# cebarker1000/heatflow

Measured on AMD Instinct MI355X. Metric: DOF-updates/s (timesteps/s x nDOF) on geballe_with_diamond, higher is better.
Workload: dtype f64

## Files before the change

heatflow_amd/csrc/heatflow_hip.hip:

```cpp

#include "hf_amg_io.hpp"

namespace {

struct MeshTables {
  std::vector<int32_t> rowptr, colidx;
  ColDict spmv;
  RowGather rg;
  std::vector<char> tag_used;
  int max_blk_nnz = 0;
};

constexpr char BLOB_MAGIC[8] = {'H', 'F', 'P', 'A', 'T', '0', '2', 0};
struct BlobHeader {
  char magic[8];
  int64_t total_bytes, nnz;
  int32_t n, ne, rba, ts, max_blk_nnz, tab_len, rg_ok, rg_max_dict, spmv_max_dict, reserved;
  int64_t count[12];
};

void steady_swap(hf_ctx* ctx) {
  hf_ctx::Steady& S = ctx->steady;
  std::swap(ctx->nbc, S.nbc); std::swap(ctx->d_bc_dofs, S.bc_dofs); std::swap(ctx->d_g, S.g);
  std::swap(ctx->nlift_rows, S.nlift_rows); std::swap(ctx->nlift, S.nlift);
// ... 393 lines not shown
  HF_TRY(dev_alloc(ctx, &F.part_rz, 2 * static_cast<size_t>(nv) * MAXP));
  HF_TRY(dev_alloc(ctx, &F.part_zz, static_cast<size_t>(nv) * MAXP));
  HF_TRY(dev_alloc(ctx, &F.part_bn, static_cast<size_t>(nv) * MAXP));
  HF_TRY(dev_alloc(ctx, &F.scal, nv));
  HF_TRY(dev_alloc(ctx, &F.red, 1));
  HF_HIP(hipMemsetAsync(F.scal, 0, sizeof(Scal) * nv, ctx->stream));
  HF_HIP(hipMemsetAsync(F.red, 0, sizeof(BRed), ctx->stream));
  if (hipHostMalloc(reinterpret_cast<void**>(&F.h_scal), sizeof(Scal) * nv) != hipSuccess) return fail(ctx, HF_ERR_ALLOC, "hipHostMalloc failed");
  const int rpb = TPB / nv;
  F.Pb = static_cast<int>(std::min<size_t>((static_cast<size_t>(ctx->n) + rpb - 1) / rpb, MAXP));
  if (F.Pb >= 64) F.Pb &= ~7;
  F.opk = 0; F.pred_iters = 0;
  F.sysA = ctx->d_M1; F.sysDinv = ctx->d_dinv1;
  F.lds = ctx->bcols.nv == nv;
  HF_HIP(hipStreamSynchronize(ctx->stream));
  F.nv = nv;
  return HF_OK;
}

int batch_flux_step(hf_ctx* ctx, int components, double rtol, int max_it, int nfs, double* out, int32_t* it_out) {
  hf_ctx::Batch& B = ctx->batch;
  hf_ctx::Batch& F = ctx->fluxnb;
  const int nv = B.nv;
  const int capd = ctx->rg_max_dict;
  const size_t sm = static_cast<size_t>(capd) * 16 + static_cast<size_t>(capd + (capd & 1)) * 8 + (RBA + 4) * 4 +
                    (static_cast<size_t>((ctx->max_blk_nnz + 1) & ~1) / 8 + 3) * 16;
  const int grid = std::min(ctx->nblk_a, 2048);
  int done = 0;
  for (int comp = 0; comp < 2; ++comp) {
    if (!((components >> comp) & 1)) continue;
    const bool second = done == 1;
    if (second) std::swap(F.u, F.uprev);
    for (int j = 0; j < nv; ++j)
      hipLaunchKernelGGL(k_grad_rows, dim3(grid), dim3(RBA), sm, ctx->stream, ctx->nblk_a, capd, ctx->d_rg_hdr,
                         reinterpret_cast<const uint4*>(ctx->d_rg_ell), reinterpret_cast<const uint4*>(ctx->d_rg_cid), ctx->d_rg_zrb,
                         ctx->d_rg_dict, ctx->d_rowptr, B.u, comp == 0 ? F.b + j : static_cast<double*>(nullptr),
                         comp == 1 ? F.b + j : static_cast<double*>(nullptr), nv, nv, j);
    HF_HIP(hipGetLastError());
    std::swap(ctx->batch, ctx->fluxnb);
    const int rc = batch_dispatch(ctx, [&](auto ops) { return decltype(ops)::pcg(ctx, false, rtol, 0.0, max_it); });
    int itmax = 0;
    for (int j = 0; j < nv; ++j) itmax = std::max(itmax, ctx->batch.h_scal[j].iters);
    std::swap(ctx->batch, ctx->fluxnb);
    if (it_out) it_out[done] = itmax;
    if (rc != HF_OK) { if (second) std::swap(F.u, F.uprev); return rc; }
    double* o = out + static_cast<size_t>(done) * nv * nfs;
    const int thr = nfs * nv;
    switch (nv) {
      case 2: hipLaunchKernelGGL((kb_gather<2>), dim3((thr + 255) / 256), dim3(256), 0, ctx->stream, nfs, ctx->d_fsamp_idx, F.u, o); break;
      case 4: hipLaunchKernelGGL((kb_gather<4>), dim3((thr + 255) / 256), dim3(256), 0, ctx->stream, nfs, ctx->d_fsamp_idx, F.u, o); break;
      case 8: hipLaunchKernelGGL((kb_gather<8>), dim3((thr + 255) / 256), dim3(256), 0, ctx->stream, nfs, ctx->d_fsamp_idx, F.u, o); break;
      default: hipLaunchKernelGGL((kb_gather<16>), dim3((thr + 255) / 256), dim3(256), 0, ctx->stream, nfs, ctx->d_fsamp_idx, F.u, o); break;
    }
    HF_HIP(hipGetLastError());
    if (second) std::swap(F.u, F.uprev);
    ++done;
  }
  return HF_OK;
}
int tangent_reset(hf_ctx* ctx) {
  hf_ctx::Batch& T = ctx->tanb;
  if (T.nv == 0) return HF_OK;
  HF_HIP(hipMemsetAsync(T.u, 0, sizeof(double) * static_cast<size_t>(ctx->n) * T.nv, ctx->stream));
  HF_HIP(hipStreamSynchronize(ctx->stream));
  T.bdf_hist = false;
  for (bool& u_ : T.pused) u_ = false;
  T.pnext = 0; T.ppending = -1;
  T.pred_iters = 0;
  return HF_OK;
}

int tangent_levels(hf_ctx* ctx) {
  hf_ctx::Batch& T = ctx->tanb;
  std::vector<int64_t> sig;
  if (ctx->precond == 1 && ctx->amg_ready)
    for (const DevLevel& L : ctx->amg) { sig.push_back(L.n); sig.push_back(L.P.ncol); }
  if (sig == ctx->tan.lev_sig) return HF_OK;
  for (auto& L : T.lev) { dev_free(&L.x); dev_free(&L.cat); if (L.own_b) dev_free(&L.b); }
  T.lev.clear();
  HF_TRY(batch_levels(ctx, T, T.nv));
  HF_HIP(hipStreamSynchronize(ctx->stream));
  ctx->tan.lev_sig = sig;
  return HF_OK;
}

int tangent_load(hf_ctx* ctx) {
  const int capd = ctx->rg_max_dict;
  const size_t sm = static_cast<size_t>(capd) * 16 + static_cast<size_t>(capd + (capd & 1)) * 8 + (RBA + 4) * 4 +
                    (static_cast<size_t>((ctx->max_blk_nnz + 1) & ~1) / 8 + 3) * 16;
  const int grid = std::min(ctx->nblk_a, 2048);
#define HF_TL(NV) hipLaunchKernelGGL(k_tangent_load<NV>, dim3(grid), dim3(RBA), sm, ctx->stream, ctx->nblk_a, capd, ctx->d_rg_hdr, \
                                     reinterpret_cast<const uint4*>(ctx->d_rg_ell), reinterpret_cast<const uint4*>(ctx->d_rg_cid), \
                                     ctx->d_rg_zrb, ctx->d_rg_dict, ctx->d_rowptr, ctx->tan.col, ctx->d_u, ctx->tan.F)
  switch (ctx->tan.nv) {
    case 2: HF_TL(2); break;
    case 4: HF_TL(4); break;
    case 8: HF_TL(8); break;
    default: HF_TL(16); break;
  }
#undef HF_TL
  HF_HIP(hipGetLastError());
  return HF_OK;
}

}

extern "C" {

const char* hf_version(void) { return "heatflow_hip 0.1 (gfx950)"; }

const char* hf_last_error(const hf_ctx* ctx) { return ctx ? ctx->err.c_str() : "null context"; }

int hf_create(int device_id, hf_ctx** out) {
  if (!out) return HF_ERR_ARG;
  *out = nullptr;
  int count = 0;
  if (hipGetDeviceCount(&count) != hipSuccess || count <= 0) return HF_ERR_HIP;
  if (device_id < 0 || device_id >= count) return HF_ERR_ARG;
  hf_ctx* ctx = new hf_ctx();
  ctx->dev = device_id;
  auto bail = [&](int rc) { *out = ctx; return rc; };
  if (hipSetDevice(device_id) != hipSuccess) return bail(fail(ctx, HF_ERR_HIP, "hipSetDevice(%d) failed", device_id));
  if (hipStreamCreateWithFlags(&ctx->stream, hipStreamNonBlocking) != hipSuccess)
    return bail(fail(ctx, HF_ERR_HIP, "hipStreamCreate failed"));
  if (hipEventCreate(&ctx->ev0) != hipSuccess || hipEventCreate(&ctx->ev1) != hipSuccess)
    return bail(fail(ctx, HF_ERR_HIP, "hipEventCreate failed"));
  if (hipHostMalloc(reinterpret_cast<void**>(&ctx->h_scal), sizeof(Scal)) != hipSuccess)
    return bail(fail(ctx, HF_ERR_ALLOC, "hipHostMalloc failed"));
  if (hipHostMalloc(reinterpret_cast<void**>(&ctx->h_mirror), sizeof(ScalMirror), hipHostMallocMapped | hipHostMallocCoherent) != hipSuccess ||
      hipHostGetDevicePointer(reinterpret_cast<void**>(&ctx->d_mirror), ctx->h_mirror, 0) != hipSuccess)
    return bail(fail(ctx, HF_ERR_ALLOC, "hipHostMalloc (mapped) failed"));
  *ctx->h_mirror = ScalMirror{};
  int rc = dev_alloc(ctx, &ctx->d_scal, 1);
  if (rc == HF_OK) rc = dev_alloc(ctx, &ctx->d_part_pAp, MAXP);
  if (rc == HF_OK) rc = dev_alloc(ctx, &ctx->d_part_rz, 2 * MAXP);
  if (rc == HF_OK) rc = dev_alloc(ctx, &ctx->d_part_zz, MAXP);
  if (rc == HF_OK) rc = dev_alloc(ctx, &ctx->d_part_bn, MAXP);
  if (rc == HF_OK && reset_scal(ctx) != HF_OK) rc = HF_ERR_HIP;
  if (rc == HF_OK) {
    hipLaunchKernelGGL(k_zero_entries, dim3(1), dim3(64), 0, ctx->stream, 0, static_cast<const int32_t*>(nullptr), static_cast<double*>(nullptr));
    if (hipStreamSynchronize(ctx->stream) != hipSuccess) rc = fail(ctx, HF_ERR_HIP, "first kernel launch failed: %s", hipGetErrorString(hipGetLastError()));
  }
  *out = ctx;
  return rc;
}

int hf_destroy(hf_ctx* ctx) {
  if (!ctx) return HF_ERR_ARG;
  (void)hipSetDevice(ctx->dev);
  if (ctx->stream) (void)hipStreamSynchronize(ctx->stream);
  dev_free(&ctx->d_zr); dev_free(&ctx->d_elem); dev_free(&ctx->d_kappa); dev_free(&ctx->d_rhoc);
  dev_free(&ctx->d_rowptr); dev_free(&ctx->d_colidx); dev_free(&ctx->d_cdict_ptr); dev_free(&ctx->d_cdict); dev_free(&ctx->d_cid); dev_free(&ctx->d_blk_eptr); dev_free(&ctx->d_blk_cptr); dev_free(&ctx->d_blk_ent); dev_free(&ctx->d_rg_hdr); dev_free(&ctx->d_rg_ell); dev_free(&ctx->d_rg_cid); dev_free(&ctx->d_rg_dict); dev_free(&ctx->d_rg_zrb); dev_free(&ctx->d_kappa_rg); dev_free(&ctx->d_rhoc_rg); dev_free(&ctx->d_M); dev_free(&ctx->d_A); dev_free(&ctx->d_dinv);
  dev_free(&ctx->d_bc_dofs); dev_free(&ctx->d_g); dev_free(&ctx->d_lift_rows); dev_free(&ctx->d_lift_ptr);
  dev_free(&ctx->d_lift_bc); dev_free(&ctx->d_lift_slot); dev_free(&ctx->d_lift_val);
  dev_free(&ctx->d_uprev); dev_free(&ctx->d_ustart);
  dev_free(&ctx->d_u); dev_free(&ctx->d_b); dev_free(&ctx->d_r); dev_free(&ctx->d_p); dev_free(&ctx->d_Ap);
  free_batch(ctx); free_batch_state(ctx->fluxb); free_batch_cols(ctx); free_amg(ctx); free_responses(ctx); proj_free(ctx); dev_free(&ctx->d_z); dev_free(&ctx->d_z2);
  steady_free(ctx); load_free(ctx); tangent_free(ctx); kt_free(ctx);
  dev_free(&ctx->d_M1); dev_free(&ctx->d_dinv1); dev_free(&ctx->d_gz); dev_free(&ctx->d_gr); dev_free(&ctx->d_bz); dev_free(&ctx->d_br);
  dev_free(&ctx->d_tmp); dev_free(&ctx->d_part_pAp); dev_free(&ctx->d_part_rz); dev_free(&ctx->d_part_zz);
  dev_free(&ctx->d_part_bn); dev_free(&ctx->d_scal); dev_free(&ctx->d_samp_idx); dev_free(&ctx->d_samp); dev_free(&ctx->d_fsamp_idx);
  for (auto& e : ctx->prof_ev) (void)hipEventDestroy(e);
  if (ctx->h_scal) (void)hipHostFree(ctx->h_scal);
  if (ctx->h_mirror) (void)hipHostFree(ctx->h_mirror);
  if (ctx->ev0) (void)hipEventDestroy(ctx->ev0);
  if (ctx->ev1) (void)hipEventDestroy(ctx->ev1);
  if (ctx->stream) (void)hipStreamDestroy(ctx->stream);
  delete ctx;
  return HF_OK;
}

int hf_set_mesh(hf_ctx* ctx, int32_t n, int32_t ne, const double* zr, const int32_t* tri, const int32_t* tag) {
  if (!ctx) return HF_ERR_ARG;
  if (!zr || !tri || !tag || n <= 0 || ne <= 0) return fail(ctx, HF_ERR_ARG, "hf_set_mesh: null pointer or empty mesh");
  HF_HIP(hipSetDevice(ctx->dev));
  int32_t maxtag = 0;
  for (int64_t k = 0; k < 3LL * ne; ++k)
    if (tri[k] < 0 || tri[k] >= n) return fail(ctx, HF_ERR_ARG, "hf_set_mesh: triangle %lld references node %d outside [0,%d)", (long long)(k / 3), tri[k], n);
  for (int32_t e = 0; e < ne; ++e) {
    if (tag[e] < 0) return fail(ctx, HF_ERR_ARG, "hf_set_mesh: negative cell tag at cell %d", e);
    maxtag = std::max(maxtag, tag[e]);
    const double* p0 = zr + 2 * tri[3 * e], *p1 = zr + 2 * tri[3 * e + 1], *p2 = zr + 2 * tri[3 * e + 2];
    const double d = (p1[0] - p0[0]) * (p2[1] - p0[1]) - (p2[0] - p0[0]) * (p1[1] - p0[1]);
    if (!(d != 0.0)) return fail(ctx, HF_ERR_ARG, "hf_set_mesh: degenerate triangle %d", e);
  }
  const auto t0 = std::chrono::steady_clock::now();
  auto lap = [&](const char* what) {
    if (std::getenv("HEATFLOW_DEBUG")) std::fprintf(stderr, "[set_mesh] %-28s %.3f s\n", what, std::chrono::duration<double>(std::chrono::steady_clock::now() - t0).count());
  };
  lap("checked");
  MeshTables T;
  Pattern P;
  HF_TRY(build_csr(ctx, n, ne, tri, P));
  lap("+ csr pattern");
  build_rowgather(n, ne, tri, tag, P);
  lap("+ row-gather lists");
  if (!build_coldict(P.rowptr, P.colidx, n, SRPC, T.spmv)) return fail(ctx, HF_ERR_ARG, "an SpMV chunk touches more than 65535 columns (16-bit positions)");
  lap("+ spmv column lists");
  T.rowptr.swap(P.rowptr);
  T.colidx.swap(P.colidx);
  T.max_blk_nnz = P.max_blk_nnz;
  T.rg = std::move(P.rg);
  T.tag_used.assign(static_cast<size_t>(maxtag) + 1, 0);
  for (int32_t e = 0; e < ne; ++e) T.tag_used[tag[e]] = 1;
  const int rc = install_mesh(ctx, n, ne, zr, tri, tag, T);
  lap("+ installed");
  return rc;
}

int hf_set_mesh_prebuilt(hf_ctx* ctx, int32_t n, int32_t ne, const double* zr, const int32_t* tri, const int32_t* tag,
                         const void* blob, int64_t bytes) {
  if (!ctx) return HF_ERR_ARG;
  if (!zr || !tri || !tag || !blob || n <= 0 || ne <= 0 || bytes <= 0) return fail(ctx, HF_ERR_ARG, "hf_set_mesh_prebuilt: null pointer or empty mesh");
  HF_HIP(hipSetDevice(ctx->dev));
  std::vector<unsigned char> staged;
  const unsigned char* src = nullptr;
  HF_TRY(blob_on_host(ctx, blob, bytes, staged, &src));
  MeshTables T;
  HF_TRY(parse_mesh_tables(ctx, src, bytes, n, ne, T));
  return install_mesh(ctx, n, ne, zr, tri, tag, T);
}

int hf_pattern_export_size(hf_ctx* ctx, int64_t* bytes) {
  if (!ctx || !bytes) return HF_ERR_ARG;
  if (!ctx->have_mesh) return fail(ctx, HF_ERR_STATE, "hf_pattern_export_size before hf_set_mesh");
  *bytes = mesh_tables_bytes(ctx);
  return HF_OK;
}

int hf_pattern_export(hf_ctx* ctx, void* blob, int64_t bytes) {
  if (!ctx || !blob) return HF_ERR_ARG;
  if (!ctx->have_mesh) return fail(ctx, HF_ERR_STATE, "hf_pattern_export before hf_set_mesh");
  if (bytes != mesh_tables_bytes(ctx)) return fail(ctx, HF_ERR_ARG, "hf_pattern_export: buffer of %lld bytes, need %lld", (long long)bytes, (long long)mesh_tables_bytes(ctx));
  HF_HIP(hipSetDevice(ctx->dev));
  std::vector<unsigned char> host(static_cast<size_t>(bytes));
  HF_TRY(write_mesh_tables(ctx, host.data()));
  HF_HIP(hipMemcpy(blob, host.data(), static_cast<size_t>(bytes), hipMemcpyDefault));
  return HF_OK;
}

int hf_set_materials(hf_ctx* ctx, int32_t n_mat, const int32_t* tags, const double* kappa, const double* rho_c) {
  if (!ctx) return HF_ERR_ARG;
  if (!ctx->have_mesh) return fail(ctx, HF_ERR_STATE, "hf_set_materials before hf_set_mesh");
  if (n_mat <= 0 || !tags || !kappa || !rho_c) return fail(ctx, HF_ERR_ARG, "hf_set_materials: bad arguments");
  HF_HIP(hipSetDevice(ctx->dev));
  std::vector<double> tk(ctx->tab_len, std::nan("")), tc(ctx->tab_len, std::nan(""));
  for (int32_t i = 0; i < n_mat; ++i) {
    if (tags[i] < 0) return fail(ctx, HF_ERR_ARG, "hf_set_materials: negative tag");
    if (!(kappa[i] > 0.0) || !(rho_c[i] > 0.0)) return fail(ctx, HF_ERR_ARG, "hf_set_materials: kappa and rho_c must be positive");
    if (tags[i] < ctx->tab_len) { tk[tags[i]] = kappa[i]; tc[tags[i]] = rho_c[i]; }
  }
  for (int t = 0; t < ctx->tab_len; ++t)
    if (ctx->h_tag_used[t] && std::isnan(tk[t])) return fail(ctx, HF_ERR_ARG, "hf_set_materials: cell tag %d has no material", t);
  HF_HIP(copy_sync(ctx, ctx->d_kappa, tk.data(), sizeof(double) * ctx->tab_len, hipMemcpyHostToDevice));
  HF_HIP(copy_sync(ctx, ctx->d_rhoc, tc.data(), sizeof(double) * ctx->tab_len, hipMemcpyHostToDevice));
  HF_TRY(upload_rg_tables(ctx, tk, &tc));
  ctx->have_mat = true;
  ctx->assembled = false;
  ctx->steady.ready = false;
  return tangent_reset(ctx);
}

int hf_update_kappa(hf_ctx* ctx, int32_t n_mat, const int32_t* tags, const double* kappa) {
  if (!ctx) return HF_ERR_ARG;
  if (!ctx->have_mat || !ctx->assembled) return fail(ctx, HF_ERR_STATE, "hf_update_kappa needs a completed hf_assemble first");
  if (n_mat <= 0 || !tags || !kappa) return fail(ctx, HF_ERR_ARG, "hf_update_kappa: bad arguments");
  HF_HIP(hipSetDevice(ctx->dev));
  std::vector<double> tk(ctx->tab_len);
  HF_HIP(copy_sync(ctx, tk.data(), ctx->d_kappa, sizeof(double) * ctx->tab_len, hipMemcpyDeviceToHost));
  for (int32_t i = 0; i < n_mat; ++i) {
    if (tags[i] < 0 || tags[i] >= ctx->tab_len || !ctx->h_tag_used[tags[i]])
      return fail(ctx, HF_ERR_ARG, "hf_update_kappa: tag %d is not a cell tag of the mesh", tags[i]);
    if (!(kappa[i] > 0.0)) return fail(ctx, HF_ERR_ARG, "hf_update_kappa: kappa must be positive");
    if (ctx->kt.on && ctx->kt.tabled[tags[i]])
      return fail(ctx, HF_ERR_ARG, "hf_update_kappa: tag %d carries a kappa(T) table (hf_set_kappa_tables)", tags[i]);
  }
  for (int32_t i = 0; i < n_mat; ++i) {
    tk[tags[i]] = kappa[i];
  }
  HF_HIP(copy_sync(ctx, ctx->d_kappa, tk.data(), sizeof(double) * ctx->tab_len, hipMemcpyHostToDevice));
  HF_TRY(upload_rg_tables(ctx, tk, nullptr));
  ctx->steady.ready = false;
  return hf_assemble(ctx, ctx->dt_step, ctx->mode);
}

int hf_set_dirichlet(hf_ctx* ctx, int32_t n_bc, const int32_t* dofs) {
  if (!ctx) return HF_ERR_ARG;
  if (!ctx->have_mesh) return fail(ctx, HF_ERR_STATE, "hf_set_dirichlet before hf_set_mesh");
  if (n_bc < 0 || (n_bc > 0 && !dofs)) return fail(ctx, HF_ERR_ARG, "hf_set_dirichlet: bad arguments");
  HF_HIP(hipSetDevice(ctx->dev));
  std::vector<char> seen(ctx->n, 0);
  for (int32_t q = 0; q < n_bc; ++q) {
    if (dofs[q] < 0 || dofs[q] >= ctx->n) return fail(ctx, HF_ERR_ARG, "hf_set_dirichlet: dof %d outside [0,%d)", dofs[q], ctx->n);
    if (seen[dofs[q]]) return fail(ctx, HF_ERR_ARG, "hf_set_dirichlet: dof %d listed twice (resolve overlaps on the host)", dofs[q]);
    seen[dofs[q]] = 1;
  }
  free_batch(ctx);
  ctx->nbc = n_bc;
  HF_TRY(dev_alloc(ctx, &ctx->d_bc_dofs, n_bc));
  HF_TRY(dev_alloc(ctx, &ctx->d_g, n_bc));
  if (n_bc > 0) HF_HIP(copy_sync(ctx, ctx->d_bc_dofs, dofs, sizeof(int32_t) * n_bc, hipMemcpyHostToDevice));
  HF_TRY(build_lift(ctx));
  free_amg(ctx);
  free_responses(ctx);
  ctx->assembled = false;
  return HF_OK;
}

int hf_assemble(hf_ctx* ctx, double dt, int32_t mode) {
  if (!ctx) return HF_ERR_ARG;
  if (!ctx->have_mesh || !ctx->have_mat) return fail(ctx, HF_ERR_STATE, "hf_assemble needs hf_set_mesh and hf_set_materials first");
  if (!(dt > 0.0)) return fail(ctx, HF_ERR_ARG, "hf_assemble: dt must be positive");
  if (mode < 0 || mode > 3) return fail(ctx, HF_ERR_ARG, "hf_assemble: unknown mode %d", mode);
  if (ctx->kt.on && mode != HF_ASM_ROW_GATHER)
    return fail(ctx, HF_ERR_ARG, "hf_assemble: kappa(T) tables are evaluated by the row-gather kernel only (HF_ASM_ROW_GATHER)");
  HF_HIP(hipSetDevice(ctx->dev));
  ctx->dt_step = dt;
  ctx->dt = ctx->scheme == HF_TIME_BDF2 ? 2.0 * dt / 3.0 : dt;
  ctx->mode = mode;
  HF_HIP(hipEventRecord(ctx->ev0, ctx->stream));
  HF_TRY(launch_assemble(ctx));
  if (ctx->kt.on) {
    HF_TRY(kt_revalue(ctx, ctx->d_u, nullptr));
  } else {
    if (ctx->nbc > 0) {
      if (ctx->nlift > 0)
        hipLaunchKernelGGL(k_take_lift, dim3((ctx->nlift + 255) / 256), dim3(256), 0, ctx->stream, ctx->nlift,
                           ctx->d_lift_slot, ctx->d_A, ctx->d_lift_val);
      hipLaunchKernelGGL(k_bc_rows, dim3((ctx->nbc + 255) / 256), dim3(256), 0, ctx->stream, ctx->nbc, ctx->d_bc_dofs,
                         ctx->d_rowptr, ctx->d_colidx, ctx->d_A);
    }
    hipLaunchKernelGGL(k_dinv, dim3((ctx->n + 255) / 256), dim3(256), 0, ctx->stream, ctx->n, ctx->d_rowptr,
                       ctx->d_colidx, ctx->d_A, ctx->d_dinv);
  }
  HF_HIP(hipEventRecord(ctx->ev1, ctx->stream));
  HF_HIP(hipGetLastError());
  HF_HIP(hipStreamSynchronize(ctx->stream));
  float ms = 0.f;
  HF_HIP(hipEventElapsedTime(&ms, ctx->ev0, ctx->ev1));
  ctx->last_ms = ms;
  if (ctx->precond == 1) {
    OperatorPrint now;
    HF_TRY(operator_print(ctx, now));
    if (!(ctx->amg_ready && ctx->amg_reuse)) {
      HF_TRY(build_amg_auto(ctx));
      ctx->amg_print = std::move(now);
    } else {
      ctx->amg_fine_stale = !same_print(now, ctx->amg_print) || ctx->kt.on;
    }
  }
  if (ctx->precond == 1 && ctx->amg_ready) {
    ctx->amg[0].A.val = ctx->d_A;
    ctx->amg[0].dinv = ctx->d_dinv;
  }
  ctx->assembled = true;
  ctx->pred_iters = 0;
  ctx->have_prev = false;
  ctx->bdf_hist = false;
  free_responses(ctx);
  return tangent_reset(ctx);
}

int hf_set_precond(hf_ctx* ctx, int32_t kind, int32_t reuse) {
  if (!ctx) return HF_ERR_ARG;
  if (kind < 0 || kind > 1) return fail(ctx, HF_ERR_ARG, "hf_set_precond: unknown preconditioner %d", kind);
  if (kind != ctx->precond) { ctx->assembled = false; ctx->pred_iters = 0; (void)hipSetDevice(ctx->dev); free_batch(ctx); }
  if (kind == 0) { (void)hipSetDevice(ctx->dev); free_amg(ctx); }
  ctx->precond = kind;
  ctx->amg_reuse = reuse ? 1 : 0;
  return HF_OK;
}

int hf_set_time_scheme(hf_ctx* ctx, int32_t scheme) {
  if (!ctx) return HF_ERR_ARG;
  if (scheme != HF_TIME_BACKWARD_EULER && scheme != HF_TIME_BDF2) return fail(ctx, HF_ERR_ARG, "hf_set_time_scheme: unknown scheme %d", scheme);
  if (scheme != ctx->scheme) {
    (void)hipSetDevice(ctx->dev);
    free_batch(ctx);
    ctx->assembled = false;
    ctx->pred_iters = 0;
    ctx->scheme = scheme;
  }
  return HF_OK;
}

int hf_set_kappa_tables(hf_ctx* ctx, int32_t n_tab, const int32_t* tags, const double* t0, const double* dT, const int32_t* n_knots,
                        const double* values, int32_t picard_sweeps) {
  if (!ctx) return HF_ERR_ARG;
  if (!ctx->have_mesh) return fail(ctx, HF_ERR_STATE, "hf_set_kappa_tables before hf_set_mesh");
  if (n_tab < 0) return fail(ctx, HF_ERR_ARG, "hf_set_kappa_tables: negative table count");
  HF_HIP(hipSetDevice(ctx->dev));
  if (n_tab == 0) {
    if (ctx->kt.on) {
      free_batch(ctx);
      ctx->assembled = false;
      ctx->pred_iters = 0;
    }
    kt_free(ctx);
    return HF_OK;
  }
  if (!tags || !t0 || !dT || !n_knots || !values) return fail(ctx, HF_ERR_ARG, "hf_set_kappa_tables: null pointer");
  if (picard_sweeps < 1 || picard_sweeps > KT_MAX_PICARD)
    return fail(ctx, HF_ERR_ARG, "hf_set_kappa_tables: picard_sweeps %d outside 1..%d", picard_sweeps, KT_MAX_PICARD);
  if (!ctx->rg_ok || (ctx->assembled && ctx->mode != HF_ASM_ROW_GATHER))
    return fail(ctx, HF_ERR_ARG, "hf_set_kappa_tables: kappa(T) is evaluated by the row-gather kernel only (HF_ASM_ROW_GATHER on a mesh with row-gather lists)");
  std::vector<KTab> hdr(64, KTab{0.0, 0.0, 0, 0});
  std::vector<double> vals;
  std::vector<char> tabled(ctx->tab_len, 0);
  for (int32_t i = 0; i < n_tab; ++i) {
    const int32_t tg = tags[i];
    if (tg < 0 || tg >= ctx->tab_len || !ctx->h_tag_used[tg]) return fail(ctx, HF_ERR_ARG, "hf_set_kappa_tables: tag %d is not a cell tag of the mesh", tg);
    if (tabled[tg]) return fail(ctx, HF_ERR_ARG, "hf_set_kappa_tables: tag %d listed twice", tg);
    if (n_knots[i] < 2 || n_knots[i] > KT_MAX_KNOTS)
      return fail(ctx, HF_ERR_ARG, "hf_set_kappa_tables: table of tag %d has %d knots (2..%d)", tg, n_knots[i], KT_MAX_KNOTS);
    if (!std::isfinite(t0[i]) || !(dT[i] > 0.0) || !std::isfinite(dT[i]) || !std::isfinite(t0[i] + (n_knots[i] - 1) * dT[i]))
      return fail(ctx, HF_ERR_ARG, "hf_set_kappa_tables: table of tag %d: T0 finite and dT > 0 needed", tg);
    tabled[tg] = 1;
    const size_t q = std::find(ctx->h_rg_tags.begin(), ctx->h_rg_tags.end(), tg) - ctx->h_rg_tags.begin();
    if (q >= ctx->h_rg_tags.size()) return fail(ctx, HF_ERR_ARG, "hf_set_kappa_tables: tag %d has no row-gather dictionary entry", tg);
    hdr[q] = KTab{t0[i], 1.0 / dT[i], n_knots[i], static_cast<int>(vals.size())};
    for (int32_t k = 0; k < n_knots[i]; ++k) {
      const double v = values[vals.size()];
      if (!(v > 0.0) || !std::isfinite(v)) return fail(ctx, HF_ERR_ARG, "hf_set_kappa_tables: value %d of the table of tag %d is not positive and finite", k, tg);
      vals.push_back(v);
    }
  }
  kt_free(ctx);
  free_batch(ctx);
  hf_ctx::KappaT& K = ctx->kt;
  HF_TRY(dev_alloc(ctx, &K.hdr, 64));
  HF_TRY(dev_alloc(ctx, &K.vals, vals.size()));
  HF_TRY(dev_alloc(ctx, &K.pic, ctx->n));
  HF_TRY(dev_alloc(ctx, &K.b0, ctx->n));
  HF_TRY(dev_alloc(ctx, &K.change, 1));
  HF_HIP(copy_sync(ctx, K.hdr, hdr.data(), sizeof(KTab) * 64, hipMemcpyHostToDevice));
  HF_HIP(copy_sync(ctx, K.vals, vals.data(), sizeof(double) * vals.size(), hipMemcpyHostToDevice));
  K.tabled = std::move(tabled);
  K.picard = picard_sweeps;
  K.on = true;
  ctx->assembled = false;
  ctx->pred_iters = 0;
  return HF_OK;
}

int hf_get_picard_change(hf_ctx* ctx, double* max_du) {
  if (!ctx || !max_du) return HF_ERR_ARG;
  if (!ctx->kt.on || !ctx->kt.have_change) return fail(ctx, HF_ERR_STATE, "hf_get_picard_change: no step with kappa(T) tables since they were set");
  HF_HIP(hipSetDevice(ctx->dev));
  unsigned long long bits = 0;
  HF_HIP(copy_sync(ctx, &bits, ctx->kt.change, sizeof bits, hipMemcpyDeviceToHost));
  std::memcpy(max_du, &bits, sizeof bits);
  return HF_OK;
}

int hf_set_start_vector(hf_ctx* ctx, int32_t kind) {
// ... 1059 lines not shown
```

heatflow_amd/csrc/hf_context.hpp:

```cpp

#pragma once
#include <hip/hip_runtime.h>
#include <hip/hip_ext.h>

#include <algorithm>
#include <chrono>
#include <cmath>
#include <cstdarg>
#include <cstdint>
#include <cstdio>
#include <cstdlib>
#include <cstring>
#include <string>
#include <thread>
#include <vector>

#include "amg_host.hpp"
#include "heatflow_hip.h"

namespace {

constexpr int RB = 256;
#ifndef HF_RBA
#define HF_RBA 256
#endif
constexpr int RBA = HF_RBA;
constexpr int TPB = 256;
constexpr int NCOL = 32;
#ifndef HF_STAGE_U
#define HF_STAGE_U 2
#endif
#ifndef HF_UNROLL
#define HF_UNROLL 4
#endif
constexpr int MAXP = 1024;
constexpr int MAXRESP = 4;
#ifndef HF_PROJ_MH
#define HF_PROJ_MH 6
#endif
constexpr int PROJ_MH = HF_PROJ_MH;
constexpr int PROJ_MT = PROJ_MH + MAXRESP;
constexpr int TS = 512;
#ifndef HF_SPMV_RPC
#define HF_SPMV_RPC 512
#endif
#ifndef HF_SPMV_UN
#define HF_SPMV_UN 8
#endif
constexpr int SRPC = HF_SPMV_RPC;

struct ScalMirror {
  double zz, bn2;
  int iters;
  int pad_;
  unsigned long long done_st;
  unsigned long long tested_st;
};
inline int mirror_tested(const ScalMirror* m, unsigned epoch) {
  const unsigned long long v = __atomic_load_n(&m->tested_st, __ATOMIC_ACQUIRE);
  return static_cast<unsigned>(v >> 32) == epoch ? static_cast<int>(v & 0xffffffffu) - 1 : -1;
}
inline int mirror_done(const ScalMirror* m, unsigned epoch) {
  const unsigned long long v = __atomic_load_n(&m->done_st, __ATOMIC_ACQUIRE);
  return static_cast<unsigned>(v >> 32) == epoch ? static_cast<int>(v & 0xffffffffu) : 0;
}

struct Scal {
  double tol2;
  double bn2;
  double zz;
  int iters;
  int done;
  int first;
  unsigned epoch;
  ScalMirror* mirror;
};

constexpr int NV_MAX = 16;
struct BRed { double pAp[NV_MAX], rz[2][NV_MAX], zz[NV_MAX], bn[NV_MAX]; };

constexpr int KT_MAX_KNOTS = 256;
constexpr int KT_MAX_PICARD = 8;
struct KTab { double t0, inv_dt; int n, off; };

}

struct hf_ctx {
  int dev = 0;
  hipStream_t stream = nullptr;
  hipEvent_t ev0 = nullptr, ev1 = nullptr;
  std::string err;
  double last_ms = 0.0;

  int32_t n = 0, ne = 0, nbc = 0;
  int64_t nnz = 0;
  int nchunks = 0, P = 0;
  int nchunks_s = 0, Ps = 0;
  int max_chunk_nnz_s = 0;
  int32_t *d_cdict_ptr = nullptr, *d_cdict = nullptr;
  uint16_t* d_cid = nullptr;
  int max_cdict = 0;
  bool cdict_own = false;
  bool c16 = true;
  bool have_mesh = false, have_mat = false, assembled = false;
  double dt = 0.0;
  double dt_step = 0.0;
  int mode = 0;
  int scheme = HF_TIME_BACKWARD_EULER;

  std::vector<int32_t> h_rowptr, h_colidx, h_tri, h_tag;
  std::vector<char> h_tag_used;
  bool owner_ready = false;

  double2* d_zr = nullptr;
  int4* d_elem = nullptr;
  int tab_len = 0;
  double *d_kappa = nullptr, *d_rhoc = nullptr;
  int32_t *d_rowptr = nullptr, *d_colidx = nullptr;
  int32_t *d_blk_eptr = nullptr, *d_blk_cptr = nullptr;
  int2* d_blk_ent = nullptr;
  int nblk_a = 0;
  int max_blk_nnz = 0, ncolors = 0;
  int64_t elist_len = 0;
  bool rg_ok = false;
  int4* d_rg_hdr = nullptr;
  uint16_t *d_rg_ell = nullptr, *d_rg_cid = nullptr;
  int32_t* d_rg_dict = nullptr;
  double2* d_rg_zrb = nullptr;
  int rg_max_dict = 0, rg_grid = 0, rg_grid_k = 0;
  int64_t n_rg_ell = 0, n_rg_dict = 0, n_cdict = 0;
  std::vector<int32_t> h_rg_tags;
  double *d_kappa_rg = nullptr, *d_rhoc_rg = nullptr;
  double *d_M = nullptr, *d_A = nullptr, *d_dinv = nullptr;
  int32_t* d_bc_dofs = nullptr;
  double* d_g = nullptr;
  int32_t nlift_rows = 0, nlift = 0;
  int32_t *d_lift_rows = nullptr, *d_lift_ptr = nullptr, *d_lift_bc = nullptr, *d_lift_slot = nullptr;
  double* d_lift_val = nullptr;
  double *d_u = nullptr, *d_b = nullptr, *d_r = nullptr, *d_p = nullptr, *d_Ap = nullptr;
  double *d_uprev = nullptr, *d_ustart = nullptr;
  bool have_prev = false;
  bool bdf_hist = false;
  int extrapolate = 1;
  int start_kind = 3;
  std::vector<double> h_g0, h_g1;
  int g_hist = 0;
  struct BcResponse { std::vector<double> dir; double* w = nullptr; };
  std::vector<BcResponse> resp;
  long long resp_solves = 0;
  struct Proj {
    double *V[PROJ_MT] = {nullptr}, *F[PROJ_MT] = {nullptr};
    bool used[PROJ_MT] = {false};
    int next = 0, pending = -1;
    double *G = nullptr, *alpha = nullptr, *part = nullptr;
    bool ready = false;
  } proj;
  double *d_tmp = nullptr;
  double *d_part_pAp = nullptr, *d_part_rz = nullptr, *d_part_zz = nullptr, *d_part_bn = nullptr;
  Scal* d_scal = nullptr;
  Scal* h_scal = nullptr;
  ScalMirror* h_mirror = nullptr;
  ScalMirror* d_mirror = nullptr;
  unsigned epoch = 0;
  int32_t* d_samp_idx = nullptr;
  double* d_samp = nullptr;
  int samp_cap = 0;
  int pred_iters = 0;
  int precond = 0;
  int amg_reuse = 0;
  bool amg_ready = false;
  struct DevCsr {
    int nrow = 0, ncol = 0, lanes = 8; int64_t nnz = 0; int32_t *ptr = nullptr, *idx = nullptr; double* val = nullptr;
    float* valf = nullptr;
    int max_row = 0;
    int rpc = 0, nchunks = 0, chunk_nnz = 0;
    int32_t *dptr = nullptr, *dict = nullptr;
    uint16_t* cid = nullptr;
    int max_dict = 0;
    int64_t ndict = 0;
  };
  struct DevLevel {
    DevCsr A, P, R, Rt, GP;
    double *dinv = nullptr, *x = nullptr, *cat = nullptr, *b = nullptr, *res = nullptr;
    bool own_b = false;
    double omega = 0; int n = 0;
  };
  std::vector<DevLevel> amg;
  double* d_coarse_inv = nullptr;
  float* d_coarse_inv_f = nullptr;
  int coarse_n = 0, coarse_ld = 0;
  bool amg_fine_stale = false;
  int amg_fuse0 = 0;
  bool amg_f32 = true;
  double amg_opc = 0.0, amg_setup_s = 0.0;
  struct OperatorPrint { double dt = 0.0; std::vector<double> kappa, rhoc; int32_t nbc = 0; uint64_t bc_hash = 0; int32_t scheme = 0; } amg_print;
  long long amg_fallbacks = 0;
  struct Steady {
    bool ready = false;
    int precond = 0, pred_iters = 0;
    int32_t nbc = 0, nlift_rows = 0, nlift = 0;
    int32_t *bc_dofs = nullptr, *lift_rows = nullptr, *lift_ptr = nullptr, *lift_bc = nullptr, *lift_slot = nullptr;
    double *g = nullptr, *lift_val = nullptr, *K = nullptr, *dinv = nullptr, *Kfree = nullptr;
    std::vector<DevLevel> amg;
    double* coarse_inv = nullptr;
    float* coarse_inv_f = nullptr;
    int coarse_n = 0, coarse_ld = 0;
    bool amg_ready = false, amg_fine_stale = false;
    double amg_opc = 0.0, amg_setup_s = 0.0;
    OperatorPrint amg_print;
  } steady;
  double* d_load = nullptr;
  bool have_load = false;
  double *d_z = nullptr, *d_z2 = nullptr;
  bool flux_ready = false;
  int flux_valid = 0;
  double *d_M1 = nullptr, *d_dinv1 = nullptr, *d_gz = nullptr, *d_gr = nullptr, *d_bz = nullptr, *d_br = nullptr;
  int pred_flux[2] = {0, 0};
  struct BatchLevel { double *x = nullptr, *cat = nullptr, *b = nullptr, *res = nullptr; bool own_b = false; };
  struct Batch {
    int nv = 0;
    int opk = 0;
    const double *sysA = nullptr, *sysDinv = nullptr;
    double *A = nullptr, *dinv = nullptr, *lift_val = nullptr;
    double *A1 = nullptr, *lift1 = nullptr;
    double delta[NV_MAX] = {};
    double *g = nullptr;
    double *u = nullptr, *uprev = nullptr, *ustart = nullptr, *b = nullptr, *r = nullptr, *p = nullptr, *Ap = nullptr;
    double *z = nullptr, *z2 = nullptr, *tmp = nullptr;
    double *part_pAp = nullptr, *part_rz = nullptr, *part_zz = nullptr, *part_bn = nullptr;
    Scal *scal = nullptr, *h_scal = nullptr;
    ScalMirror *h_mirror = nullptr, *d_mirror = nullptr;
    unsigned epoch = 0;
    BRed* red = nullptr;
    std::vector<BatchLevel> lev;
    int Pb = 0, pred_iters = 0;
    bool have_prev = false;
    bool bdf_hist = false;
    double *pV[PROJ_MH] = {nullptr}, *pF[PROJ_MH] = {nullptr}, *pG = nullptr, *palpha = nullptr, *ppart = nullptr;
    bool pused[PROJ_MH] = {false};
    int pnext = 0, ppending = -1;
    unsigned loaded = 0;
    bool lds = false;
    const double* load = nullptr;
  } batch;
  struct BatchCols {
    int nv = 0, rpc = 0, nchunks = 0, cap_nnz = 0, cap_dict = 0;
    int32_t *ptr = nullptr, *dict = nullptr, *own = nullptr;
    uint16_t* id = nullptr;
  } bcols;
  Batch fluxb;
  Batch fluxnb;
  int32_t* d_fsamp_idx = nullptr;
  Batch tanb;
  struct Tangent {
    bool ready = false;
    int npar = 0, nv = 0;
    int32_t* col = nullptr;
    double* F = nullptr;
    bool steady_state = false;
    std::vector<int64_t> lev_sig;
  } tan;
  int fsamp_cap = 0;
  struct KappaT {
    bool on = false;
    int picard = 1;
    KTab* hdr = nullptr;
    double* vals = nullptr;
    std::vector<char> tabled;
    double *pic = nullptr, *b0 = nullptr;
    unsigned long long* change = nullptr;
    bool have_change = false;
    int grid = 0;
  } kt;
  bool prof = false;
  std::vector<hipEvent_t> prof_ev;
  int prof_used = 0, prof_base = 0;
  double prof_spmv_ms = 0.0;
  long long prof_spmv_n = 0;
};

namespace {

int fail(hf_ctx* c, int code, const char* fmt, ...);
inline size_t pad16(size_t b) { return (b + 15) & ~static_cast<size_t>(15); }

inline void cpu_relax() {
#if defined(__x86_64__) || defined(__i386__)
  __builtin_ia32_pause();
#else
  std::this_thread::yield();
#endif
}

hipError_t copy_sync(hf_ctx* ctx, void* dst, const void* src, size_t bytes, hipMemcpyKind kind) {
  if (bytes == 0) return hipSuccess;
  const hipError_t e = hipMemcpyAsync(dst, src, bytes, kind, ctx->stream);
  return e != hipSuccess ? e : hipStreamSynchronize(ctx->stream);
}

int fail(hf_ctx* c, int code, const char* fmt, ...) {
  char buf[512];
  va_list ap;
  va_start(ap, fmt);
  vsnprintf(buf, sizeof buf, fmt, ap);
  va_end(ap);
  if (c) c->err = buf;
// ... 38 lines not shown
```

heatflow_amd/csrc/hf_kernels.hpp:

```cpp
#pragma once
#include "hf_context.hpp"

namespace {


template <int NW = 4>
__device__ __forceinline__ double block_sum(double v, double* sw) {
#pragma unroll
  for (int o = 32; o > 0; o >>= 1) v += __shfl_down(v, o, 64);
  const int w = threadIdx.x >> 6;
  if ((threadIdx.x & 63) == 0) sw[w] = v;
  __syncthreads();
  double t = sw[0];
#pragma unroll
  for (int k = 1; k < NW; ++k) t += sw[k];
  __syncthreads();
  return t;
}

__device__ __forceinline__ double sum_partials(const double* __restrict__ part, int P, double* s4) {
  double v = 0.0;
  for (int k = threadIdx.x; k < P; k += TPB) v += part[k];
  return block_sum(v, s4);
}
// ... 485 lines not shown
          const ElemRow r = element_row(Pi, Pj, Pk, rhoc_idx[tg], kappa);
          dA += fma(dt, r.k0, r.m0);
          sA[base + pj] += fma(dt, r.k1, r.m1);
          sA[base + pk] += fma(dt, r.k2, r.m2);
        }
      }
      sA[base + pd] = dA;
    }
    __syncthreads();
    for (int k = t; k < cA.y; k += RBA) {
      Av[cA.x + k] = sA[k];
      sA[k] = 0.0;
    }
    blk = nxt;
  }
}

__global__ __launch_bounds__(TPB) void k_max_abs_diff(int n, const double* __restrict__ a, const double* __restrict__ b,
                                                      unsigned long long* __restrict__ out) {
  __shared__ double s[TPB];
  double m = 0.0;
  for (int i = blockIdx.x * TPB + threadIdx.x; i < n; i += gridDim.x * TPB) m = fmax(m, fabs(a[i] - b[i]));
  s[threadIdx.x] = m;
  __syncthreads();
  for (int h = TPB / 2; h > 0; h >>= 1) {
    if (threadIdx.x < h) s[threadIdx.x] = fmax(s[threadIdx.x], s[threadIdx.x + h]);
    __syncthreads();
  }
  if (threadIdx.x == 0) atomicMax(out, static_cast<unsigned long long>(__double_as_longlong(s[0])));
}

__global__ __launch_bounds__(TPB) void k_eval_state(int n, const double* __restrict__ u, const double* __restrict__ uprev,
                                                    double* __restrict__ out) {
#pragma clang fp contract(off)
  for (int i = blockIdx.x * TPB + threadIdx.x; i < n; i += gridDim.x * TPB) out[i] = uprev ? 2.0 * u[i] - uprev[i] : u[i];
}

__global__ void k_gather_coords(int64_t total, const int32_t* __restrict__ dict, const double2* __restrict__ zr,
                                double2* __restrict__ zrb) {
  const int64_t i = static_cast<int64_t>(blockIdx.x) * blockDim.x + threadIdx.x;
  if (i < total) zrb[i] = zr[dict[i]];
}

__global__ __launch_bounds__(TPB) void k_assemble_global(int ne, const int32_t* __restrict__ rowptr,
                                                         const int32_t* __restrict__ colidx,
                                                         const int4* __restrict__ elem,
                                                         const double2* __restrict__ zr,
                                                         const double* __restrict__ kappa_tab,
                                                         const double* __restrict__ rhoc_tab, double dt,
                                                         double* __restrict__ Mv, double* __restrict__ Av) {
  const int e = blockIdx.x * TPB + threadIdx.x;
  if (e >= ne) return;
  const int4 el = elem[e];
  const int nd[3] = {el.x, el.y, el.z};
  double m[6], kk[6], av6[6];
  element_local(zr[el.x], zr[el.y], zr[el.z], rhoc_tab[el.w], kappa_tab[el.w], m, kk);
#pragma unroll
  for (int q = 0; q < 6; ++q) av6[q] = fma(dt, kk[q], m[q]);
#pragma unroll
  for (int a = 0; a < 3; ++a) {
    const int s0 = rowptr[nd[a]], s1 = rowptr[nd[a] + 1];
#pragma unroll
    for (int b = 0; b < 3; ++b) {
      int s = s0;
      while (s < s1 && colidx[s] != nd[b]) ++s;
      const int q = sym_index(a, b);
      atomicAdd(&Mv[s], m[q]);
      atomicAdd(&Av[s], av6[q]);
    }
  }
}

__global__ __launch_bounds__(RBA) void k_grad_rhs(int n, const int32_t* __restrict__ blk_eptr,
                                                  const int2* __restrict__ blk_ent, const double2* __restrict__ zr,
                                                  const double* __restrict__ u, double* __restrict__ bz,
                                                  double* __restrict__ br) {
  __shared__ double sB[2 * RBA];
  const int blk = blockIdx.x;
  const int r0 = blk * RBA;
  const int r1 = min(n, r0 + RBA);
  for (int k = threadIdx.x; k < 2 * RBA; k += RBA) sB[k] = 0.0;
  __syncthreads();
  for (int q = blk_eptr[blk] + threadIdx.x; q < blk_eptr[blk + 1]; q += RBA) {
#pragma clang fp contract(off)
    const AsmEntry e = load_entry(blk_ent, q);
    const double2 p0 = zr[e.n0], p1 = zr[e.n1], p2 = zr[e.n2];
    const double u0 = u[e.n0], u1 = u[e.n1], u2 = u[e.n2];
    const double d = (p1.x - p0.x) * (p2.y - p0.y) - (p2.x - p0.x) * (p1.y - p0.y);
    const double area = 0.5 * fabs(d);
    const double gz = (u0 * (p1.y - p2.y) + u1 * (p2.y - p0.y) + u2 * (p0.y - p1.y)) / d;
    const double gr = (u0 * (p2.x - p1.x) + u1 * (p0.x - p2.x) + u2 * (p1.x - p0.x)) / d;
    const double rsum = (p0.y + p1.y) + p2.y;
    const double wgt[3] = {area * (p0.y + rsum) / 12.0, area * (p1.y + rsum) / 12.0, area * (p2.y + rsum) / 12.0};
    const int nd[3] = {e.n0, e.n1, e.n2};
    const unsigned owned = (e.w3 >> 8) & 7u;
#pragma unroll
    for (int a = 0; a < 3; ++a) {
      if (!((owned >> a) & 1u)) continue;
      atomicAdd(&sB[2 * (nd[a] - r0)], gz * wgt[a]);
      atomicAdd(&sB[2 * (nd[a] - r0) + 1], gr * wgt[a]);
    }
  }
  __syncthreads();
  for (int k = threadIdx.x; k < r1 - r0; k += RBA) {
    bz[r0 + k] = sB[2 * k];
    br[r0 + k] = sB[2 * k + 1];
  }
}

__global__ void k_take_lift(int nlift, const int32_t* __restrict__ slot, double* __restrict__ A,
                            double* __restrict__ val) {
  const int q = blockIdx.x * blockDim.x + threadIdx.x;
  if (q >= nlift) return;
  val[q] = A[slot[q]];
  A[slot[q]] = 0.0;
}

__global__ void k_bc_rows(int nbc, const int32_t* __restrict__ dofs, const int32_t* __restrict__ rowptr,
                          const int32_t* __restrict__ colidx, double* __restrict__ A) {
  const int q = blockIdx.x * blockDim.x + threadIdx.x;
  if (q >= nbc) return;
  const int row = dofs[q];
  for (int k = rowptr[row]; k < rowptr[row + 1]; ++k) A[k] = (colidx[k] == row) ? 1.0 : 0.0;
}

__global__ void k_dinv(int n, const int32_t* __restrict__ rowptr, const int32_t* __restrict__ colidx,
                       const double* __restrict__ A, double* __restrict__ dinv) {
  const int row = blockIdx.x * blockDim.x + threadIdx.x;
  if (row >= n) return;
  double d = 0.0;
  for (int k = rowptr[row]; k < rowptr[row + 1]; ++k)
    if (colidx[k] == row) d = A[k];
  dinv[row] = 1.0 / d;
}

__global__ void k_lift(int nrows, const int32_t* __restrict__ rows, const int32_t* __restrict__ ptr,
                       const int32_t* __restrict__ bc, const double* __restrict__ val,
                       const double* __restrict__ g, double* __restrict__ b) {
  const int q = blockIdx.x * blockDim.x + threadIdx.x;
  if (q >= nrows) return;
  double s = 0.0;
  for (int k = ptr[q]; k < ptr[q + 1]; ++k) s += val[k] * g[bc[k]];
  b[rows[q]] -= s;
}

__global__ void k_set_bc(int nbc, const int32_t* __restrict__ dofs, const double* __restrict__ g,
                         double* __restrict__ b, double* __restrict__ u) {
  const int q = blockIdx.x * blockDim.x + threadIdx.x;
  if (q >= nbc) return;
  b[dofs[q]] = g[q];
  u[dofs[q]] = g[q];
}

__global__ void k_gather(int ns, const int32_t* __restrict__ idx, const double* __restrict__ u,
                         double* __restrict__ out) {
  const int q = blockIdx.x * blockDim.x + threadIdx.x;
  if (q < ns) out[q] = u[idx[q]];
}

__global__ __launch_bounds__(TPB) void k_hold_load(int n, const int32_t* __restrict__ rowptr, const int32_t* __restrict__ colidx,
                                                   const double* __restrict__ K, const double* __restrict__ u,
                                                   const unsigned char* __restrict__ mask, double* __restrict__ F) {
  const int row = blockIdx.x * blockDim.x + threadIdx.x;
  if (row >= n) return;
  double s = 0.0;
  if (!mask[row])
    for (int k = rowptr[row]; k < rowptr[row + 1]; ++k) s += K[k] * u[colidx[k]];
  F[row] = s;
}

__global__ void k_mark_rows(int nq, const int32_t* __restrict__ idx, unsigned char* __restrict__ mask) {
  const int q = blockIdx.x * blockDim.x + threadIdx.x;
  if (q < nq) mask[idx[q]] = 1;
}

__device__ __forceinline__ unsigned long long mirror_stamp(unsigned epoch, int v) {
  return (static_cast<unsigned long long>(epoch) << 32) | static_cast<unsigned>(v);
}
__device__ __forceinline__ void mirror_publish(ScalMirror* m, double zz, int iters, int done, unsigned epoch) {
  if (m == nullptr) return;
  m->zz = zz;
  m->iters = iters;
  __hip_atomic_store(&m->done_st, mirror_stamp(epoch, done), __ATOMIC_RELAXED, __HIP_MEMORY_SCOPE_SYSTEM);
  __threadfence_system();
  __hip_atomic_store(&m->tested_st, mirror_stamp(epoch, iters + 1), __ATOMIC_RELEASE, __HIP_MEMORY_SCOPE_SYSTEM);
}
__device__ __forceinline__ void mirror_breakdown(ScalMirror* m, unsigned epoch) {
  if (m != nullptr) __hip_atomic_store(&m->done_st, mirror_stamp(epoch, 2), __ATOMIC_RELEASE, __HIP_MEMORY_SCOPE_SYSTEM);
}

struct ColComp { const int32_t* dptr; const int32_t* dict; const uint16_t* id; int xd_off; int own; };

#ifndef HF_NT_STREAM
#define HF_NT_STREAM 0
#endif
#ifndef HF_PIPE
#define HF_PIPE 1
#endif
#ifndef HF_PHASE_CLOCK
#define HF_PHASE_CLOCK -1
#endif
#if HF_PHASE_CLOCK >= 0
#ifndef HF_PHASE_CONV
#define HF_PHASE_CONV 0
#endif
__device__ unsigned long long g_phase[MAXP * 16];
#define HF_STAMP(slot)                                                                                   \
  do {                                                                                                   \
    if (MODE == HF_PHASE_CLOCK && C16 && (MODE != 0 || (part2 != nullptr) == (HF_PHASE_CONV != 0)) && threadIdx.x == 0 && (slot) < 16) \
      g_phase[blockIdx.x * 16 + (slot)] = wall_clock64();                                                \
  } while (0)
#else
#define HF_STAMP(slot) do { } while (0)
#endif
template <typename T>
__device__ __forceinline__ T stream_load(const T* p) {
#if HF_NT_STREAM
  return __builtin_nontemporal_load(p);
#else
  return *p;
#endif
}

__device__ __forceinline__ double bdf2_operand(double un, double unm1) { return (4.0 * un - unm1) * (1.0 / 3.0); }

template <int MODE, bool C16 = false, typename VT = double, int UN = 8>
__global__ __launch_bounds__(TS) __attribute__((amdgpu_waves_per_eu(8, 8))) void k_spmv(int n, int nchunks, int rpc ,
                                              const int32_t* __restrict__ rowptr, const int32_t* __restrict__ colidx,
                                              const VT* __restrict__ vals, const double* __restrict__ x,
                                              double* __restrict__ y, Scal* __restrict__ scal,
                                              double* __restrict__ part0, const double* __restrict__ bvec,
                                              const double* __restrict__ dinv, double* __restrict__ pvec,
                                              double* __restrict__ part1, double* __restrict__ part2, double w,
                                              int npart ,
                                              int parity, ColComp comp) {
  extern __shared__ double sprod[];
  __shared__ double s4[TS / 64];
  __shared__ int s_own;
  constexpr bool BDF = MODE >= 12 && MODE <= 15;
  auto opnd = [&](int c) { return BDF ? bdf2_operand(x[c], bvec[c]) : x[c]; };
  if ((MODE == 3 || MODE == 4 || MODE == 6 || MODE == 9) && scal->done) return;
  if ((MODE == 0 || MODE == 7) && scal != nullptr && scal->done) return;
  double acc0 = 0.0, acc1 = 0.0, acc2 = 0.0;
  double beta = 0.0;
  bool first9 = false;
  if (MODE == 9) {
    first9 = scal->first != 0;
    if (!first9) {
      double v0 = 0.0, v1 = 0.0, v2 = 0.0;
      for (int k = threadIdx.x; k < npart; k += TS) {
        v0 += part1[parity * MAXP + k];
        v1 += part1[(parity ^ 1) * MAXP + k];
        v2 += part2[k];
      }
      const double rz_new = block_sum<TS / 64>(v0, s4);
      const double rz_old = block_sum<TS / 64>(v1, s4);
      const double zz = block_sum<TS / 64>(v2, s4);
      const bool conv = zz <= scal->tol2;
      if (blockIdx.x == 0 && threadIdx.x == 0) {
        scal->zz = zz;
        if (conv) scal->done = 1;
      }
      if (conv) return;
      beta = rz_new / rz_old;
    }
  }
  auto cycle_gate = [&]() {
    if (!((MODE == 3 || MODE == 0) && part2 != nullptr)) return false;
    double v2 = 0.0;
    for (int k = threadIdx.x; k < npart; k += TS) v2 += part2[k];
    const double zz = block_sum<TS / 64>(v2, s4);
    const bool conv = zz <= scal->tol2;
    if (blockIdx.x == 0 && threadIdx.x == 0) {
      if (conv) { scal->zz = zz; scal->done = 1; }
      mirror_publish(scal->mirror, zz, scal->iters, conv ? 1 : 0, scal->epoch);
    }
    return conv;
  };
  constexpr bool PIPELINED = C16 && (HF_PIPE == 2 || (HF_PIPE == 1 && sizeof(VT) == 4));
  if (!PIPELINED && cycle_gate()) return;
  const ChunkIter sched(nchunks);
  HF_STAMP(0);
  int stamp_at = 1;
  (void)stamp_at;
  const int tpr = (MODE == 0 || MODE == 6 || MODE == 7) ? TS / rpc : 1;
  const int prel = static_cast<int>(threadIdx.x) / tpr;
  const int psub = static_cast<int>(threadIdx.x) % tpr;
  struct RowOps { double b, d, y, p, x; };
  auto row_operands = [&](int prc, bool from_slice) {
    RowOps e{0.0, 0.0, 0.0, 0.0, 0.0};
    if (MODE == 2 || MODE == 3 || MODE == 4 || MODE == 5 || MODE == 7 || MODE == 8 || MODE == 11 || MODE == 13 || MODE == 15) e.b = bvec[prc];
    if (MODE == 2 || MODE == 4 || MODE == 5 || MODE == 10 || MODE == 11 || MODE == 14 || MODE == 15) e.d = dinv[prc];
    if (MODE == 6 || (MODE == 9 && !first9)) e.y = y[prc];
    if (MODE == 9 && !first9) e.p = pvec[prc];
    if ((MODE == 4 || MODE == 8 || MODE == 9 || MODE == 11) && !from_slice) e.x = x[prc];
    if (BDF) e.x = x[prc];
    return e;
  };
  auto rows_phase = [&](bool pin, int prow, int pa, int pb, const RowOps& e) {
    if ((MODE == 0 || MODE == 6 || MODE == 7) && tpr > 1) {
      double s = 0.0;
      if (pin)
        for (int j = pa + psub; j < pb; j += tpr) s += sprod[j];
      for (int o = tpr >> 1; o > 0; o >>= 1) s += __shfl_down(s, o, 64);
      if (pin && psub == 0) {
        y[prow] = (MODE == 6) ? e.y + s : s;
        if (MODE == 7) acc0 += e.b * s;
      }
    } else if (pin) {
      const int row = prow;
      double s = 0.0;
      for (int j = pa; j < pb; ++j) s += sprod[j];
      if (MODE == 0) {
        y[row] = s;
      } else if (MODE == 2) {
        const double ri = e.b - s;
        const double zi = e.d * ri;
        y[row] = ri;
        pvec[row] = zi;
        acc0 += ri * zi;
        acc1 += zi * zi;
        acc2 += (e.d * e.b) * (e.d * e.b);
      } else if (MODE == 3) {
        y[row] = e.b - s;
      } else if (MODE == 4) {
        const double yi = e.x + w * e.d * (e.b - s);
        y[row] = yi;
        acc0 += e.b * yi;
      } else if (MODE == 5) {
        const double ri = e.b - s;
        y[row] = ri;
        pvec[row] = w * e.d * ri;
        acc1 += (e.d * ri) * (e.d * ri);
        acc2 += (e.d * e.b) * (e.d * e.b);
      } else if (MODE == 7) {
        y[row] = s;
        acc0 += e.b * s;
      } else if (MODE == 6) {
        y[row] = e.y + s;
      } else if (MODE == 8) {
        y[row] = s;
        pvec[row] = 2.0 * e.x - e.b;
      } else if (MODE == 10) {
        y[row] = s + w * e.d;
      } else if (MODE == 11) {
        y[row] = s + w * e.d;
        pvec[row] = 2.0 * e.x - e.b;
      } else if (BDF) {
        y[row] = (MODE == 14 || MODE == 15) ? s + w * e.d : s;
        pvec[row] = (MODE == 13 || MODE == 15) ? 2.0 * e.x - e.b : e.x;
      } else {
        const double api = first9 ? s : s + beta * e.y;
        const double pi = first9 ? e.x : e.x + beta * e.p;
        y[row] = api;
        pvec[row] = pi;
        acc0 += pi * api;
      }
    }
  };
  if (PIPELINED) {
    struct Bounds { int k0, k1, d0, d1; };
    auto bounds = [&](int ch) {
      Bounds q;
      const int a0 = ch * rpc, a1 = min(n, a0 + rpc);
      q.k0 = rowptr[a0]; q.k1 = rowptr[a1];
      q.d0 = comp.dptr[ch]; q.d1 = comp.dptr[ch + 1];
      return q;
    };
    int lhead[HF_STAGE_U];
    double v[UN];
    int id[UN];
    auto heads = [&](const Bounds& q, bool live) {
      const int dl = max(q.d1 - 1, 0), kl = max(q.k1 - 1, 0);
      const int t = static_cast<int>(threadIdx.x);
#pragma unroll
      for (int u = 0; u < HF_STAGE_U; ++u) lhead[u] = comp.dict[min(q.d0 + (live ? t + u * TS : (t & 31)), dl)];
      __builtin_amdgcn_sched_barrier(0);
#pragma unroll
      for (int u = 0; u < UN; ++u) {
        const int kk = min(q.k0 + (live ? t + u * TS : (t & 31)), kl);
        v[u] = static_cast<double>(stream_load(&vals[kk]));
        id[u] = static_cast<int>(stream_load(&comp.id[kk]));
      }
    };
    double* xd = sprod + comp.xd_off;
    Bounds cur = bounds(min(sched.chunk, nchunks - 1));
    heads(cur, sched.chunk < sched.end);
    if (cycle_gate()) return;
    for (int chunk = sched.chunk; chunk < sched.end; chunk += sched.step) {
      const bool more = chunk + sched.step < sched.end;
      const int r0 = chunk * rpc, r1 = min(n, r0 + rpc);
      const int k0 = cur.k0, k1 = cur.k1, d0 = cur.d0, nd = cur.d1 - cur.d0;
      const int prow = r0 + prel;
      const bool pin = prow < r1;
      const int prc = min(prow, r1 - 1);
      int c0[HF_STAGE_U];
      double x0[HF_STAGE_U];
#pragma unroll
      for (int u = 0; u < HF_STAGE_U; ++u) { c0[u] = lhead[u]; x0[u] = opnd(c0[u]); }
      const Bounds nxt = bounds(more ? chunk + sched.step : chunk);
      const int pa = rowptr[prc] - k0, pb = rowptr[prc + 1] - k0;
      RowOps e = row_operands(prc, comp.own != 0);
#pragma unroll
      for (int u = 0; u < HF_STAGE_U; ++u) {
        const int i = static_cast<int>(threadIdx.x) + u * TS;
        if (i < nd) {
          xd[i] = x0[u];
          if ((MODE == 4 || MODE == 8 || MODE == 9 || MODE == 11) && c0[u] == r0) s_own = i;
        }
      }
      for (int i = threadIdx.x + HF_STAGE_U * TS; i < nd; i += HF_STAGE_U * TS) {
        int c[HF_STAGE_U];
        double xv[HF_STAGE_U];
#pragma unroll
        for (int u = 0; u < HF_STAGE_U; ++u) c[u] = comp.dict[d0 + min(i + u * TS, nd - 1)];
#pragma unroll
        for (int u = 0; u < HF_STAGE_U; ++u) xv[u] = opnd(c[u]);
#pragma unroll
        for (int u = 0; u < HF_STAGE_U; ++u)
          if (i + u * TS < nd) {
            xd[i + u * TS] = xv[u];
            if ((MODE == 4 || MODE == 8 || MODE == 9 || MODE == 11) && c[u] == r0) s_own = i + u * TS;
          }
      }
      __syncthreads();
      HF_STAMP(stamp_at); ++stamp_at;
      if ((MODE == 4 || MODE == 8 || MODE == 9 || MODE == 11) && comp.own && pin) e.x = xd[s_own + (prow - r0)];
#pragma unroll
      for (int u = 0; u < UN; ++u) {
        const int kk = k0 + static_cast<int>(threadIdx.x) + u * TS;
        if (kk < k1) sprod[kk - k0] = v[u] * xd[id[u]];
      }
      for (int kb = k0 + UN * TS; kb < k1; kb += UN * TS) {
#pragma unroll
        for (int u = 0; u < UN; ++u) {
          const int kk = min(kb + static_cast<int>(threadIdx.x) + u * TS, k1 - 1);
          v[u] = static_cast<double>(stream_load(&vals[kk]));
          id[u] = static_cast<int>(stream_load(&comp.id[kk]));
        }
#pragma unroll
        for (int u = 0; u < UN; ++u) {
          const int kk = kb + static_cast<int>(threadIdx.x) + u * TS;
          if (kk < k1) sprod[kk - k0] = v[u] * xd[id[u]];
        }
      }
      heads(nxt, more);
      __syncthreads();
      HF_STAMP(stamp_at); ++stamp_at;
      rows_phase(pin, prow, pa, pb, e);
      __syncthreads();
      HF_STAMP(stamp_at); ++stamp_at;
      cur = nxt;
    }
  } else {
  const ChunkIter& sched_ = sched;
  for (int chunk = sched_.chunk; chunk < sched_.end; chunk += sched_.step) {
    const int r0 = chunk * rpc;
    const int r1 = min(n, r0 + rpc);
    const int k0 = rowptr[r0];
    const int k1 = rowptr[r1];
    const int prow = r0 + prel;
    const bool pin = prow < r1;
    int pa = 0, pb = 0;
    if (pin) {
      pa = rowptr[prow] - k0;
      pb = rowptr[prow + 1] - k0;
    }
    RowOps e = row_operands(min(prow, r1 - 1), C16 && comp.own != 0);
    if (C16) {
      double* xd = sprod + comp.xd_off;
      const int d0 = comp.dptr[chunk], nd = comp.dptr[chunk + 1] - d0;
      int k = k0 + threadIdx.x;
      double v[HF_UNROLL];
      int id[HF_UNROLL];
#pragma unroll
      for (int u = 0; u < HF_UNROLL; ++u) {
        const bool in = k + u * TS < k1;
        v[u] = in ? static_cast<double>(stream_load(&vals[k + u * TS])) : 0.0;
        id[u] = in ? static_cast<int>(stream_load(&comp.id[k + u * TS])) : 0;
      }
      for (int i = threadIdx.x; i < nd; i += HF_STAGE_U * TS) {
        int c[HF_STAGE_U];
        double xv[HF_STAGE_U];
#pragma unroll
        for (int u = 0; u < HF_STAGE_U; ++u) c[u] = (i + u * TS < nd) ? comp.dict[d0 + i + u * TS] : 0;
#pragma unroll
        for (int u = 0; u < HF_STAGE_U; ++u) xv[u] = (i + u * TS < nd) ? opnd(c[u]) : 0.0;
#pragma unroll
        for (int u = 0; u < HF_STAGE_U; ++u)
          if (i + u * TS < nd) {
            xd[i + u * TS] = xv[u];
            if ((MODE == 4 || MODE == 8 || MODE == 9 || MODE == 11) && c[u] == r0) s_own = i + u * TS;
          }
      }
      __syncthreads();
      HF_STAMP(stamp_at); ++stamp_at;
      if ((MODE == 4 || MODE == 8 || MODE == 9 || MODE == 11) && comp.own && pin) e.x = xd[s_own + (prow - r0)];
      while (k < k1) {
        const int kn = k + HF_UNROLL * TS;
        double vn[HF_UNROLL];
        int idn[HF_UNROLL];
#pragma unroll
        for (int u = 0; u < HF_UNROLL; ++u) {
          const bool in = kn + u * TS < k1;
          vn[u] = in ? static_cast<double>(stream_load(&vals[kn + u * TS])) : 0.0;
          idn[u] = in ? static_cast<int>(stream_load(&comp.id[kn + u * TS])) : 0;
        }
#pragma unroll
        for (int u = 0; u < HF_UNROLL; ++u)
          if (k + u * TS < k1) sprod[k - k0 + u * TS] = v[u] * xd[id[u]];
#pragma unroll
        for (int u = 0; u < HF_UNROLL; ++u) { v[u] = vn[u]; id[u] = idn[u]; }
        k = kn;
      }
    } else {
      for (int k = k0 + threadIdx.x; k < k1; k += HF_UNROLL * TS) {
        int c[HF_UNROLL];
        double v[HF_UNROLL], xv[HF_UNROLL];
#pragma unroll
        for (int u = 0; u < HF_UNROLL; ++u) {
          const bool in = k + u * TS < k1;
          c[u] = in ? colidx[k + u * TS] : 0;
          v[u] = in ? static_cast<double>(vals[k + u * TS]) : 0.0;
        }
#pragma unroll
        for (int u = 0; u < HF_UNROLL; ++u) xv[u] = (k + u * TS < k1) ? opnd(c[u]) : 0.0;
#pragma unroll
        for (int u = 0; u < HF_UNROLL; ++u)
          if (k + u * TS < k1) sprod[k - k0 + u * TS] = v[u] * xv[u];
      }
    }
    __syncthreads();
    HF_STAMP(stamp_at); ++stamp_at;
    rows_phase(pin, prow, pa, pb, e);
    __syncthreads();
    HF_STAMP(stamp_at); ++stamp_at;
  }
  }
  if (MODE == 2 || MODE == 7 || MODE == 9 || (MODE == 4 && part0 != nullptr)) {
    const double t0 = block_sum<TS / 64>(acc0, s4);
    if (threadIdx.x == 0) {
      part0[blockIdx.x] = t0;
      for (int q = blockIdx.x + gridDim.x; q < npart; q += gridDim.x) part0[q] = 0.0;
    }
  }
  if (MODE == 2 || MODE == 5) {
    const double t1 = block_sum<TS / 64>(acc1, s4);
    const double t2 = block_sum<TS / 64>(acc2, s4);
    if (threadIdx.x == 0) {
      part1[blockIdx.x] = t1;
      part2[blockIdx.x] = t2;
      for (int q = blockIdx.x + gridDim.x; q < npart; q += gridDim.x) { part1[q] = 0.0; part2[q] = 0.0; }
    }
  }
}

__global__ __launch_bounds__(TPB) void k_pcg_begin(int P, double rtol, double atol, const double* __restrict__ part_zz,
                                                   const double* __restrict__ part_bn, Scal* __restrict__ scal, unsigned epoch) {
  __shared__ double s4[4];
  const double zz = sum_partials(part_zz, P, s4);
  const double bn2 = sum_partials(part_bn, P, s4);
  if (threadIdx.x == 0) {
    const double tol = fmax(rtol * sqrt(bn2 > 0.0 ? bn2 : zz), atol);
    scal->tol2 = tol * tol;
    scal->bn2 = bn2;
    scal->zz = zz;
    scal->iters = 0;
    scal->first = 1;
    scal->done = (zz <= tol * tol) ? 1 : 0;
    scal->epoch = epoch;
    if (scal->mirror != nullptr) scal->mirror->bn2 = bn2;
    mirror_publish(scal->mirror, zz, 0, scal->done, epoch);
  }
}

__global__ __launch_bounds__(TPB) void k_pcg_update(int n, int nchunks, int P, int parity, Scal* __restrict__ scal,
                                                    const double* __restrict__ part_pAp, double* __restrict__ part_rz,
                                                    double* __restrict__ part_zz, double* __restrict__ x,
                                                    double* __restrict__ r, const double* __restrict__ p,
                                                    const double* __restrict__ Ap, const double* __restrict__ dinv,
                                                    double* __restrict__ z) {
  __shared__ double s4[4];
  if (scal->done) return;
  const double pAp = sum_partials(part_pAp, P, s4);
  const double rz = sum_partials(part_rz + parity * MAXP, P, s4);
  if (!(pAp > 0.0)) {
    if (blockIdx.x == 0 && threadIdx.x == 0) {
      scal->done = 2;
      mirror_breakdown(scal->mirror, scal->epoch);
    }
    return;
  }
  if (blockIdx.x == 0 && threadIdx.x == 0) { scal->iters += 1; scal->first = 0; }
  const double alpha = rz / pAp;
  double a_rz = 0.0, a_zz = 0.0;
  const ChunkIter sched(nchunks);
  for (int chunk = sched.chunk; chunk < sched.end; chunk += sched.step) {
    const int i = chunk * RB + threadIdx.x;
    if (i < n) {
      const double ri = r[i] - alpha * Ap[i];
      const double zi = dinv[i] * ri;
      x[i] += alpha * p[i];
      r[i] = ri;
      z[i] = zi;
      a_rz += ri * zi;
      a_zz += zi * zi;
    }
  }
  const double t0 = block_sum(a_rz, s4);
  const double t1 = block_sum(a_zz, s4);
  if (threadIdx.x == 0) {
    part_rz[(parity ^ 1) * MAXP + blockIdx.x] = t0;
    part_zz[blockIdx.x] = t1;
  }
}

template <int LANES, int VMODE, typename VT = double>
__global__ __launch_bounds__(TPB) void k_spmv_vec(int nrow, const int32_t* __restrict__ ptr,
                                                  const int32_t* __restrict__ idx, const VT* __restrict__ val,
                                                  const double* __restrict__ x, double* __restrict__ y,
                                                  const Scal* __restrict__ scal) {
  if (scal->done) return;
  const int lane = threadIdx.x % LANES;
  const int rows_per_pass = (gridDim.x * TPB) / LANES;
  for (int row = (blockIdx.x * TPB + threadIdx.x) / LANES; row < nrow; row += rows_per_pass) {
    const int k1 = ptr[row + 1];
    const double y0 = (VMODE == 1 && lane == 0) ? y[row] : 0.0;
    double s = 0.0;
    for (int k = ptr[row] + lane; k < k1; k += 4 * LANES) {
      int c[4];
      double v[4], xv[4];
#pragma unroll
      for (int u = 0; u < 4; ++u) {
        const bool in = k + u * LANES < k1;
        c[u] = in ? idx[k + u * LANES] : 0;
        v[u] = in ? static_cast<double>(val[k + u * LANES]) : 0.0;
      }
#pragma unroll
      for (int u = 0; u < 4; ++u) xv[u] = (k + u * LANES < k1) ? x[c[u]] : 0.0;
#pragma unroll
      for (int u = 0; u < 4; ++u) s += v[u] * xv[u];
    }
#pragma unroll
    for (int o = LANES / 2; o > 0; o >>= 1) s += __shfl_down(s, o, LANES);
    if (lane == 0) y[row] = (VMODE == 1) ? y0 + s : s;
  }
}

template <int VMODE, typename VT = double>
__global__ __launch_bounds__(TPB) void k_spmv_row(int nrow, const int32_t* __restrict__ ptr,
                                                  const int32_t* __restrict__ idx, const VT* __restrict__ val,
                                                  const double* __restrict__ x, double* __restrict__ y,
                                                  const Scal* __restrict__ scal) {
  __shared__ double s4[TPB / 64];
  if (scal->done) return;
  for (int row = blockIdx.x; row < nrow; row += gridDim.x) {
    const int k1 = ptr[row + 1];
    const double y0 = (VMODE == 1 && threadIdx.x == 0) ? y[row] : 0.0;
    double s = 0.0;
    for (int k = ptr[row] + threadIdx.x; k < k1; k += 4 * TPB) {
      int c[4];
      double v[4], xv[4];
#pragma unroll
      for (int u = 0; u < 4; ++u) {
        const bool in = k + u * TPB < k1;
        c[u] = in ? idx[k + u * TPB] : 0;
        v[u] = in ? static_cast<double>(val[k + u * TPB]) : 0.0;
      }
#pragma unroll
      for (int u = 0; u < 4; ++u) xv[u] = (k + u * TPB < k1) ? x[c[u]] : 0.0;
#pragma unroll
      for (int u = 0; u < 4; ++u) s += v[u] * xv[u];
    }
    const double t = block_sum<TPB / 64>(s, s4);
    if (threadIdx.x == 0) y[row] = (VMODE == 1) ? y0 + t : t;
  }
}

struct RespArgs { const double* w[MAXRESP]; double c[MAXRESP]; int k; };
__global__ __launch_bounds__(TPB) void k_start_vector(int n, const double* __restrict__ base, RespArgs a,
                                                      double* __restrict__ u) {
  for (int i = blockIdx.x * TPB + threadIdx.x; i < n; i += gridDim.x * TPB) {
    double s = base[i];
    for (int k = 0; k < a.k; ++k) s += a.c[k] * a.w[k][i];
    u[i] = s;
  }
}

struct ProjVecs { const double* V[PROJ_MT]; int slot[PROJ_MT]; int m; };

__global__ __launch_bounds__(TPB) void k_proj_dots(int n, ProjVecs a, const double* __restrict__ f, const double* __restrict__ Fnew,
                                                   double* __restrict__ part ) {
  __shared__ double sw[TPB / 64][2 * PROJ_MT];
  double ah[PROJ_MT], ag[PROJ_MT];
#pragma unroll
  for (int k = 0; k < PROJ_MT; ++k) { ah[k] = 0.0; ag[k] = 0.0; }
  const int stride = gridDim.x * TPB;
  for (int i = blockIdx.x * TPB + threadIdx.x; i < n; i += 2 * stride) {
    const int i2 = i + stride;
    const bool two = i2 < n;
    const double fi = f ? f[i] : 0.0, gi = Fnew ? Fnew[i] : 0.0;
    const double fj = (f && two) ? f[i2] : 0.0, gj = (Fnew && two) ? Fnew[i2] : 0.0;
    double v0[PROJ_MT], v1[PROJ_MT];
#pragma unroll
    for (int k = 0; k < PROJ_MT; ++k) {
      v0[k] = k < a.m ? a.V[k][i] : 0.0;
      v1[k] = (k < a.m && two) ? a.V[k][i2] : 0.0;
    }
#pragma unroll
    for (int k = 0; k < PROJ_MT; ++k) {
      ah[k] += v0[k] * fi;
      ag[k] += v0[k] * gi;
      ah[k] += v1[k] * fj;
      ag[k] += v1[k] * gj;
    }
  }
  const int lane = threadIdx.x & 63, wave = threadIdx.x >> 6;
#pragma unroll
  for (int k = 0; k < PROJ_MT; ++k)
    if (k < a.m) {
      double th = ah[k], tg = ag[k];
#pragma unroll
      for (int o = 32; o > 0; o >>= 1) { th += __shfl_down(th, o, 64); tg += __shfl_down(tg, o, 64); }
      if (lane == 0) { sw[wave][2 * k] = th; sw[wave][2 * k + 1] = tg; }
    }
  __syncthreads();
  if (static_cast<int>(threadIdx.x) < 2 * a.m) {
    double t = sw[0][threadIdx.x];
#pragma unroll
    for (int w = 1; w < TPB / 64; ++w) t += sw[w][threadIdx.x];
    part[threadIdx.x * MAXP + blockIdx.x] = t;
  }
}

static_assert(PROJ_MT * PROJ_MT <= 1024, "k_proj_solve holds one matrix entry per thread");
constexpr int PROJ_SOLVE_T = 1024;
__global__ __launch_bounds__(PROJ_SOLVE_T) void k_proj_solve(int P, ProjVecs a, int jnew, int do_solve, double* __restrict__ part,
                                                    double* __restrict__ G , double* __restrict__ alpha) {
  __shared__ double sh[PROJ_MT], sg[PROJ_MT];
  __shared__ double A[PROJ_MT][PROJ_MT + 1], bb[PROJ_MT], dd[PROJ_MT], xx[PROJ_MT];
  __shared__ int perm[PROJ_MT], piv, stop, rank_s;
  __shared__ double pmax;
  part += static_cast<size_t>(blockIdx.x) * 2 * PROJ_MT * MAXP;
  G += blockIdx.x * PROJ_MT * PROJ_MT;
  alpha += blockIdx.x * (PROJ_MT + 1);
  const int m = a.m, t = threadIdx.x, lane = t & 63, wave = t >> 6;
  for (int q = wave; q < 2 * m; q += PROJ_SOLVE_T / 64) {
    double v = 0.0;
    for (int k0 = 0; k0 < P; k0 += 256) {
      double e[4];
#pragma unroll
      for (int u = 0; u < 4; ++u) { const int k = k0 + lane + 64 * u; e[u] = k < P ? part[q * MAXP + k] : 0.0; }
      v += (e[0] + e[1]) + (e[2] + e[3]);
    }
#pragma unroll
    for (int o = 32; o > 0; o >>= 1) v += __shfl_down(v, o, 64);
    if (lane == 0) { if (q & 1) sg[q >> 1] = v; else sh[q >> 1] = v; }
  }
  __syncthreads();
  if (jnew >= 0 && t < m) { G[a.slot[t] * PROJ_MT + jnew] = sg[t]; G[jnew * PROJ_MT + a.slot[t]] = sg[t]; }
  if (!do_solve) return;
  __syncthreads();
  if (t < PROJ_MT + 1) alpha[t] = 0.0;
  if (t < m) {
    double gii = (jnew >= 0 && a.slot[t] == jnew) ? sg[t] : G[a.slot[t] * PROJ_MT + a.slot[t]];
    const bool ok = gii > 0.0 && gii < 1e300;
    dd[t] = ok ? 1.0 / sqrt(gii) : 0.0;
    perm[t] = t;
    xx[t] = 0.0;
  }
  __syncthreads();
  const int i = t / PROJ_MT, j = t % PROJ_MT;
  if (i < m && j < m) {
    double gij;
    if (jnew >= 0 && a.slot[j] == jnew) gij = sg[i];
    else if (jnew >= 0 && a.slot[i] == jnew) gij = sg[j];
    else gij = G[a.slot[i] * PROJ_MT + a.slot[j]];
    const bool ok = dd[i] > 0.0 && dd[j] > 0.0;
    A[i][j] = ok ? gij * dd[i] * dd[j] : (i == j ? 0.0 : 0.0);
  }
  if (t < m) bb[t] = sh[t] * dd[t];
  if (t == 0) { rank_s = 0; stop = 0; }
  __syncthreads();
  for (int c = 0; c < m; ++c) {
    if (t == 0) {
      int pi = c;
      double best = A[c][c];
      for (int q = c + 1; q < m; ++q)
        if (A[q][q] > best) { best = A[q][q]; pi = q; }
      if (c == 0) pmax = best;
      piv = pi;
      stop = !(best > 1e-12 * pmax) || !(best > 0.0);
    }
    __syncthreads();
    if (stop) break;
    const int pv = piv;
    if (pv != c) {
      if (t < m) { const double x0 = A[c][t]; A[c][t] = A[pv][t]; A[pv][t] = x0; }
      __syncthreads();
      if (t < m) { const double x0 = A[t][c]; A[t][c] = A[t][pv]; A[t][pv] = x0; }
      if (t == 0) {
        const double x0 = bb[c]; bb[c] = bb[pv]; bb[pv] = x0;
        const int p0 = perm[c]; perm[c] = perm[pv]; perm[pv] = p0;
      }
      __syncthreads();
    }
    if (i > c && i < m && j > c && j < m) A[i][j] -= A[i][c] / A[c][c] * A[c][j];
    if (i > c && i < m && j == c) bb[i] -= A[i][c] / A[c][c] * bb[c];
    if (t == 0) rank_s = c + 1;
    __syncthreads();
  }
  if (t != 0) return;
  const int rank = rank_s;
  for (int c = rank - 1; c >= 0; --c) {
    double v = bb[c];
    for (int q = c + 1; q < rank; ++q) v -= A[c][q] * xx[q];
    xx[c] = v / A[c][c];
  }
  bool finite = true;
  for (int c = 0; c < rank; ++c) finite = finite && (fabs(xx[c]) < 1e300);
  if (!finite) return;
  for (int c = 0; c < rank; ++c) alpha[a.slot[perm[c]]] = xx[c] * dd[perm[c]];
  alpha[PROJ_MT] = static_cast<double>(rank);
}

__global__ __launch_bounds__(TPB) void k_proj_combine(int n, ProjVecs a, const double* __restrict__ alpha, double* __restrict__ u) {
  double c[PROJ_MT];
#pragma unroll
  for (int k = 0; k < PROJ_MT; ++k) c[k] = k < a.m ? alpha[a.slot[k]] : 0.0;
  const int stride = gridDim.x * TPB;
  for (int i = blockIdx.x * TPB + threadIdx.x; i < n; i += 2 * stride) {
    const int i2 = i + stride;
    const bool two = i2 < n;
    double v0[PROJ_MT], v1[PROJ_MT];
#pragma unroll
    for (int k = 0; k < PROJ_MT; ++k) {
      v0[k] = k < a.m ? a.V[k][i] : 0.0;
      v1[k] = (k < a.m && two) ? a.V[k][i2] : 0.0;
    }
    double s0 = 0.0, s1 = 0.0;
#pragma unroll
    for (int k = 0; k < PROJ_MT; ++k) { s0 += c[k] * v0[k]; s1 += c[k] * v1[k]; }
// ... 241 lines not shown
```

heatflow_amd/csrc/hf_pattern.hpp:

```cpp
#pragma once
#include <thread>

#include "hf_kernels.hpp"

namespace {

struct ColDict {
  std::vector<int32_t> ptr, dict;
  std::vector<uint16_t> id;
  int max_dict = 0;
};

struct RowGather {
  bool ok = false;
  std::vector<int4> hdr;
  std::vector<uint16_t> ell;
  std::vector<int32_t> tags;
  ColDict cols;
};

struct OwnerLists {
  std::vector<int32_t> blk_eptr, blk_cptr, blk_elist;
  std::vector<int2> blk_ent;
  int ncolors = 0;
// ... 197 lines not shown
    for (int32_t i = r0; i < r1; ++i)
      for (int32_t q = nptr[i]; q < nptr[i + 1]; ++q) {
        const int32_t e = nlist[q];
        if (stamp[e] != b) { stamp[e] = b; list.push_back(e); }
      }
    std::sort(list.begin(), list.end());
    std::fill(mask.begin(), mask.end(), 0u);
    color.resize(list.size());
    int counts[NCOL] = {0};
    for (size_t k = 0; k < list.size(); ++k) {
      const int32_t e = list[k];
      uint32_t used = 0;
      for (int a = 0; a < 3; ++a) {
        const int32_t v = tri[3 * e + a];
        if (v >= r0 && v < r1) used |= mask[v - r0];
      }
      if (used == 0xFFFFFFFFu) return fail(ctx, HF_ERR_ARG, "more than %d elements share a node", NCOL);
      const int c = __builtin_ctz(~used);
      color[k] = c;
      counts[c]++;
      O.ncolors = std::max(O.ncolors, c + 1);
      for (int a = 0; a < 3; ++a) {
        const int32_t v = tri[3 * e + a];
        if (v >= r0 && v < r1) mask[v - r0] |= (1u << c);
      }
    }
    const int32_t base = static_cast<int32_t>(O.blk_elist.size());
    int32_t* cp = &O.blk_cptr[static_cast<size_t>(b) * (NCOL + 1)];
    cp[0] = base;
    for (int c = 0; c < NCOL; ++c) cp[c + 1] = cp[c] + counts[c];
    O.blk_elist.resize(O.blk_elist.size() + list.size());
    int32_t cur[NCOL];
    for (int c = 0; c < NCOL; ++c) cur[c] = cp[c];
    for (size_t k = 0; k < list.size(); ++k) O.blk_elist[cur[color[k]]++] = list[k];
    O.blk_eptr[b] = base;
    O.blk_eptr[b + 1] = static_cast<int32_t>(O.blk_elist.size());
  }
  O.blk_ent.resize(3 * O.blk_elist.size());
  for (int b = 0; b < nblk; ++b) {
    const int32_t r0 = b * RBA, r1 = std::min<int32_t>(n, r0 + RBA);
    for (int32_t q = O.blk_eptr[b]; q < O.blk_eptr[b + 1]; ++q) {
      const int32_t e = O.blk_elist[q];
      const int32_t nd[3] = {tri[3 * e], tri[3 * e + 1], tri[3 * e + 2]};
      uint32_t pos[9] = {0}, owned = 0;
      for (int a = 0; a < 3; ++a) {
        if (nd[a] < r0 || nd[a] >= r1) continue;
        owned |= 1u << a;
        const int32_t* rb = &P.colidx[P.rowptr[nd[a]]];
        const int32_t* re = &P.colidx[P.rowptr[nd[a] + 1]];
        if (re - rb > 255) return fail(ctx, HF_ERR_ARG, "row %d holds more than 255 entries", nd[a]);
        for (int c = 0; c < 3; ++c) pos[a * 3 + c] = static_cast<uint32_t>(std::lower_bound(rb, re, nd[c]) - rb);
      }
      if (tag[e] >= (1 << 21)) return fail(ctx, HF_ERR_ARG, "cell tag %d does not fit the packed list entry (max 2^21 - 1)", tag[e]);
      const uint32_t w3 = pos[8] | (owned << 8) | (static_cast<uint32_t>(tag[e]) << 11);
      O.blk_ent[3 * q] = make_int2(nd[0], nd[1]);
      O.blk_ent[3 * q + 1] = make_int2(nd[2], static_cast<int>(w3));
      O.blk_ent[3 * q + 2] = make_int2(static_cast<int>(pos[0] | (pos[1] << 8) | (pos[2] << 16) | (pos[3] << 24)),
                                       static_cast<int>(pos[4] | (pos[5] << 8) | (pos[6] << 16) | (pos[7] << 24)));
    }
  }
  return HF_OK;
}

int ensure_owner_lists(hf_ctx* ctx) {
  if (ctx->owner_ready) return HF_OK;
  if (ctx->h_tri.empty()) return fail(ctx, HF_ERR_STATE, "element lists requested without a host copy of the mesh");
  Pattern P;
  HF_TRY(build_csr(ctx, ctx->n, ctx->ne, ctx->h_tri.data(), P));
  OwnerLists O;
  HF_TRY(build_owner_lists(ctx, ctx->n, ctx->ne, ctx->h_tri.data(), ctx->h_tag.data(), P, O));
  ctx->ncolors = O.ncolors;
  ctx->elist_len = static_cast<int64_t>(O.blk_elist.size());
  HF_TRY(dev_alloc(ctx, &ctx->d_blk_eptr, O.blk_eptr.size()));
  HF_TRY(dev_alloc(ctx, &ctx->d_blk_cptr, O.blk_cptr.size()));
  HF_TRY(dev_alloc(ctx, &ctx->d_blk_ent, O.blk_ent.size()));
  HF_HIP(copy_sync(ctx, ctx->d_blk_eptr, O.blk_eptr.data(), sizeof(int32_t) * O.blk_eptr.size(), hipMemcpyHostToDevice));
  HF_HIP(copy_sync(ctx, ctx->d_blk_cptr, O.blk_cptr.data(), sizeof(int32_t) * O.blk_cptr.size(), hipMemcpyHostToDevice));
  HF_HIP(copy_sync(ctx, ctx->d_blk_ent, O.blk_ent.data(), sizeof(int2) * O.blk_ent.size(), hipMemcpyHostToDevice));
  ctx->owner_ready = true;
  return HF_OK;
}

size_t spmv_smem_bytes(const hf_ctx* c) { return static_cast<size_t>(c->max_chunk_nnz_s + (c->c16 ? c->max_cdict : 0)) * 8; }

int launch_assemble_lds(hf_ctx* ctx, bool colored, const double* kappa_tab, const double* rhoc_tab, double dt,
                        double* Mout, double* Aout) {
  HF_TRY(ensure_owner_lists(ctx));
  const int cap = (ctx->max_blk_nnz + 1) & ~1;
  const size_t sm = static_cast<size_t>(cap) * 16 + (RBA + 1) * 4;
  if (sm > 64 * 1024) {
    HF_HIP(hipFuncSetAttribute(reinterpret_cast<const void*>(&k_assemble_lds<true>),
                               hipFuncAttributeMaxDynamicSharedMemorySize, static_cast<int>(sm)));
    HF_HIP(hipFuncSetAttribute(reinterpret_cast<const void*>(&k_assemble_lds<false>),
                               hipFuncAttributeMaxDynamicSharedMemorySize, static_cast<int>(sm)));
  }
  if (colored)
    hipLaunchKernelGGL(k_assemble_lds<true>, dim3(ctx->nblk_a), dim3(RBA), sm, ctx->stream, ctx->n, cap, ctx->d_rowptr,
                       ctx->d_blk_eptr, ctx->d_blk_cptr, ctx->d_blk_ent, ctx->d_zr, kappa_tab, rhoc_tab, dt, Mout, Aout);
  else
    hipLaunchKernelGGL(k_assemble_lds<false>, dim3(ctx->nblk_a), dim3(RBA), sm, ctx->stream, ctx->n, cap, ctx->d_rowptr,
                       ctx->d_blk_eptr, ctx->d_blk_cptr, ctx->d_blk_ent, ctx->d_zr, kappa_tab, rhoc_tab, dt, Mout, Aout);
  HF_HIP(hipGetLastError());
  return HF_OK;
}

size_t rowgather_smem_bytes(int max_blk_nnz, int max_dict) {
  const size_t cap = static_cast<size_t>((max_blk_nnz + 1) & ~1);
  return cap * 16 + static_cast<size_t>(max_dict) * 16 + (RBA + 4) * 4 + (cap / 8 + 3) * 16;
}

template <bool KONLY = false>
int launch_assemble_rows(hf_ctx* ctx, const double* kappa_idx, const double* rhoc_idx, double dt, double* Mout, double* Aout) {
  const int cap = (ctx->max_blk_nnz + 1) & ~1;
  const int capd = ctx->rg_max_dict;
  const size_t sm = rowgather_smem_bytes(ctx->max_blk_nnz, capd);
  const void* fn = reinterpret_cast<const void*>(&k_assemble_rows<KONLY>);
  int& grid = KONLY ? ctx->rg_grid_k : ctx->rg_grid;
  if (grid == 0) {
    if (sm > 64 * 1024) HF_HIP(hipFuncSetAttribute(fn, hipFuncAttributeMaxDynamicSharedMemorySize, static_cast<int>(sm)));
    int per_cu = 0, ncu = 0;
    HF_HIP(hipOccupancyMaxActiveBlocksPerMultiprocessor(&per_cu, fn, RBA, sm));
    HF_HIP(hipDeviceGetAttribute(&ncu, hipDeviceAttributeMultiprocessorCount, ctx->dev));
    grid = std::max(1, std::min(ctx->nblk_a, std::max(1, per_cu) * std::max(1, ncu)));
  }
  hipLaunchKernelGGL(k_assemble_rows<KONLY>, dim3(grid), dim3(RBA), sm, ctx->stream, ctx->nblk_a, cap, capd, ctx->d_rowptr,
                     ctx->d_rg_hdr, reinterpret_cast<const uint4*>(ctx->d_rg_ell), reinterpret_cast<const uint4*>(ctx->d_rg_cid),
                     ctx->d_rg_zrb, kappa_idx, rhoc_idx, dt, Mout, Aout);
  HF_HIP(hipGetLastError());
  return HF_OK;
}

int launch_assemble(hf_ctx* ctx) {
  if (ctx->mode == HF_ASM_ROW_GATHER && ctx->rg_ok)
    return launch_assemble_rows(ctx, ctx->d_kappa_rg, ctx->d_rhoc_rg, ctx->dt, ctx->d_M, ctx->d_A);
  if (ctx->mode == HF_ASM_ROW_GATHER)
    return launch_assemble_lds(ctx, true, ctx->d_kappa, ctx->d_rhoc, ctx->dt, ctx->d_M, ctx->d_A);
  if (ctx->mode == HF_ASM_LDS_COLORED || ctx->mode == HF_ASM_LDS_ATOMIC) {
    return launch_assemble_lds(ctx, ctx->mode == HF_ASM_LDS_COLORED, ctx->d_kappa, ctx->d_rhoc, ctx->dt, ctx->d_M, ctx->d_A);
  } else {
    HF_HIP(hipMemsetAsync(ctx->d_M, 0, sizeof(double) * ctx->nnz, ctx->stream));
    HF_HIP(hipMemsetAsync(ctx->d_A, 0, sizeof(double) * ctx->nnz, ctx->stream));
    hipLaunchKernelGGL(k_assemble_global, dim3((ctx->ne + TPB - 1) / TPB), dim3(TPB), 0, ctx->stream, ctx->ne,
                       ctx->d_rowptr, ctx->d_colidx, ctx->d_elem, ctx->d_zr, ctx->d_kappa, ctx->d_rhoc, ctx->dt,
                       ctx->d_M, ctx->d_A);
  }
  HF_HIP(hipGetLastError());
  return HF_OK;
}

template <int MODE, typename VT = double>
void launch_spmv(hf_ctx* c, const VT* vals, const double* x, double* y, double* part0 = nullptr,
                 const double* bvec = nullptr, double* pvec = nullptr, double* part1 = nullptr,
                 double* part2 = nullptr, double w = 0.0, const double* dinv = nullptr, hipEvent_t ev_start = nullptr,
                 hipEvent_t ev_stop = nullptr, int parity = 0) {
  const ColComp comp{c->d_cdict_ptr, c->d_cdict, c->d_cid, c->max_chunk_nnz_s, c->cdict_own ? 1 : 0};
#define HF_SPMV_ARGS c->n, c->nchunks_s, static_cast<int>(SRPC), static_cast<const int32_t*>(c->d_rowptr),                    \
                     static_cast<const int32_t*>(c->d_colidx), vals, x, y, (MODE == 0 ? nullptr : c->d_scal), part0, bvec,  \
                     dinv ? dinv : static_cast<const double*>(c->d_dinv), pvec, part1, part2, w, c->P, parity, comp
  const std::uint32_t smem = static_cast<std::uint32_t>(spmv_smem_bytes(c));
  if (c->c16) {
    if (ev_start != nullptr) hipExtLaunchKernelGGL((k_spmv<MODE, true, VT, HF_SPMV_UN>), dim3(c->Ps), dim3(TS), smem, c->stream, ev_start, ev_stop, 0u, HF_SPMV_ARGS);
    else hipLaunchKernelGGL((k_spmv<MODE, true, VT, HF_SPMV_UN>), dim3(c->Ps), dim3(TS), smem, c->stream, HF_SPMV_ARGS);
  } else {
    if (ev_start != nullptr) hipExtLaunchKernelGGL((k_spmv<MODE, false, VT>), dim3(c->Ps), dim3(TS), smem, c->stream, ev_start, ev_stop, 0u, HF_SPMV_ARGS);
    else hipLaunchKernelGGL((k_spmv<MODE, false, VT>), dim3(c->Ps), dim3(TS), smem, c->stream, HF_SPMV_ARGS);
  }
#undef HF_SPMV_ARGS
}

constexpr int PROF_PAIRS = 64;

struct LinSys { const double* A; const double* dinv; double* x; const double* b; };

void launch_pcg_iteration(hf_ctx* c, const LinSys& s, int parity) {
  const bool timed = c->prof && c->prof_used < PROF_PAIRS;
  hipEvent_t e0 = timed ? c->prof_ev[2 * c->prof_used] : nullptr, e1 = timed ? c->prof_ev[2 * c->prof_used + 1] : nullptr;
  launch_spmv<9>(c, s.A, c->d_z, c->d_Ap, c->d_part_pAp, nullptr, c->d_p, c->d_part_rz, c->d_part_zz, 0.0, nullptr, e0, e1,
                 parity);
  if (timed) c->prof_used++;
  hipLaunchKernelGGL(k_pcg_update, dim3(c->P), dim3(TPB), 0, c->stream, c->n, c->nchunks, c->P, parity, c->d_scal,
                     c->d_part_pAp, c->d_part_rz, c->d_part_zz, s.x, c->d_r, c->d_p, c->d_Ap, s.dinv, c->d_z);
}

}
```

heatflow_amd/csrc/hf_solver.hpp:

```cpp
#pragma once
#include "hf_pattern.hpp"

namespace {

using DevCsr = hf_ctx::DevCsr;
using DevLevel = hf_ctx::DevLevel;

void free_dev_csr(DevCsr& m) { dev_free(&m.ptr); dev_free(&m.idx); dev_free(&m.val); dev_free(&m.valf); dev_free(&m.dptr); dev_free(&m.dict); dev_free(&m.cid); m = DevCsr(); }

void free_amg(hf_ctx* ctx) {
  for (size_t l = 0; l < ctx->amg.size(); ++l) {
    DevLevel& L = ctx->amg[l];
    if (l > 0) { free_dev_csr(L.A); dev_free(&L.dinv); dev_free(&L.x); dev_free(&L.cat); }
    if (L.own_b) dev_free(&L.b);
    free_dev_csr(L.P); free_dev_csr(L.R); free_dev_csr(L.Rt); free_dev_csr(L.GP);
  }
  ctx->amg.clear();
  dev_free(&ctx->d_coarse_inv);
  dev_free(&ctx->d_coarse_inv_f);
  ctx->coarse_n = 0;
  ctx->amg_ready = false;
}

int lanes_for_avg(double avg) {
// ... 88 lines not shown
  prm.fuse_fine_down_only = ctx->amg_fuse0 == 2;
}

int upload_host_levels(hf_ctx* ctx, const amg::Hierarchy& H, size_t base) {
  const bool f32 = ctx->amg_f32;
  const size_t nl = ctx->amg.size();
  for (size_t k = 0; k < H.levels.size(); ++k) {
    const size_t l = base + k;
    DevLevel& L = ctx->amg[l];
    const amg::Level& hl = H.levels[k];
    L.n = static_cast<int>(hl.dinv.size());
    L.omega = hl.omega;
    if (l == 0) {
      if (nl > 1 && hl.Rt.nrow > 0) {
        HF_TRY(upload_csr(ctx, hl.Rt, L.Rt, f32));
        if (hl.GP.nrow > 0) HF_TRY(upload_csr(ctx, hl.GP, L.GP, f32));
      }
    } else {
      HF_TRY(upload_csr(ctx, hl.A, L.A));
      HF_TRY(dev_alloc(ctx, &L.dinv, L.n));
      HF_HIP(copy_sync(ctx, L.dinv, hl.dinv.data(), sizeof(double) * L.n, hipMemcpyHostToDevice));
      if (l + 1 < nl) {
        HF_TRY(upload_csr(ctx, hl.Rt, L.Rt, f32));
        HF_TRY(upload_csr(ctx, hl.GP, L.GP, f32));
      }
    }
    if (l + 1 < nl) {
      HF_TRY(upload_csr(ctx, hl.P, L.P, f32));
      HF_TRY(upload_csr(ctx, hl.R, L.R, f32, !(l == 0 && hl.Rt.nrow > 0) || ctx->amg_reuse != 0));
    }
  }
  return HF_OK;
}

int dense_inverse(hf_ctx* ctx, int nc, const int32_t* ptr, const int32_t* idx, const double* val, double* inv) {
  const int ld = (nc + 3) & ~3;
  const int64_t nnz = ptr[nc];
  for (int i = 0; i < nc; ++i)
    for (int k = ptr[i]; k < ptr[i + 1]; ++k)
      if (idx[k] < 0 || idx[k] >= nc) return fail(ctx, HF_ERR_ARG, "coarsest operator: column %d outside [0,%d)", idx[k], nc);
  DevTemp<double> t_w, t_r, t_val;
  DevTemp<int32_t> t_ptr, t_idx;
  HF_TRY(dev_alloc(ctx, &t_w.p, static_cast<size_t>(nc) * 2 * nc));
  HF_TRY(dev_alloc(ctx, &t_r.p, static_cast<size_t>(GJ_B) * nc));
  HF_TRY(dev_alloc(ctx, &t_ptr.p, static_cast<size_t>(nc) + 1));
  HF_TRY(dev_alloc(ctx, &t_idx.p, std::max<size_t>(nnz, 1)));
  HF_TRY(dev_alloc(ctx, &t_val.p, std::max<size_t>(nnz, 1)));
  HF_HIP(copy_sync(ctx, t_ptr.p, ptr, sizeof(int32_t) * (static_cast<size_t>(nc) + 1), hipMemcpyHostToDevice));
  if (nnz > 0) {
    HF_HIP(copy_sync(ctx, t_idx.p, idx, sizeof(int32_t) * nnz, hipMemcpyHostToDevice));
    HF_HIP(copy_sync(ctx, t_val.p, val, sizeof(double) * nnz, hipMemcpyHostToDevice));
  }
  HF_HIP(hipMemsetAsync(t_w.p, 0, sizeof(double) * nc * 2 * nc, ctx->stream));
  hipLaunchKernelGGL(k_gjb_fill, dim3((nc + 255) / 256), dim3(256), 0, ctx->stream, nc, t_ptr.p, t_idx.p, t_val.p, t_w.p);
  const int tiles = (nc + 63) / 64;
  for (int c0 = 0; c0 < nc; c0 += GJ_B) {
    const int bsz = std::min(GJ_B, nc - c0);
    hipLaunchKernelGGL(k_gjb_rows, dim3(std::max(1, std::min((nc + TPB - 1) / TPB, 64))), dim3(TPB), 0, ctx->stream, nc, c0, bsz, t_w.p, t_r.p);
    hipLaunchKernelGGL(k_gjb_update, dim3(tiles, tiles), dim3(TPB), 0, ctx->stream, nc, c0, bsz, t_w.p, t_r.p);
  }
  HF_HIP(hipGetLastError());
  HF_HIP(hipMemsetAsync(inv, 0, sizeof(double) * nc * ld, ctx->stream));
  HF_HIP(hipMemcpy2DAsync(inv, sizeof(double) * ld, t_w.p + nc, sizeof(double) * 2 * nc, sizeof(double) * nc, nc,
                          hipMemcpyDeviceToDevice, ctx->stream));
  HF_HIP(hipStreamSynchronize(ctx->stream));
  return HF_OK;
}

int finish_amg(hf_ctx* ctx, const amg::Csr& Ac, int coarse_n, double op_complexity, const std::chrono::steady_clock::time_point t0) {
  const bool f32 = ctx->amg_f32;
  const size_t nl = ctx->amg.size();
  auto lap = [&](const char* what) {
    if (std::getenv("HEATFLOW_DEBUG")) std::fprintf(stderr, "[amg setup] %-28s %.3f s\n", what, std::chrono::duration<double>(std::chrono::steady_clock::now() - t0).count());
  };
  {
    DevLevel& L = ctx->amg[0];
    if (L.Rt.nrow > 0 && (L.Rt.rpc == 0 || (L.GP.nrow > 0 && L.GP.rpc == 0))) {
      free_dev_csr(L.Rt);
      free_dev_csr(L.GP);
    }
  }
  if (std::getenv("HEATFLOW_DEBUG")) {
    auto show = [](const char* nm, size_t l, const DevCsr& m) {
      if (m.nrow) std::fprintf(stderr, "[amg] level %zu %-2s %8d x %8d nnz %9lld (%.1f/row, max %d) %s rpc %d lanes %d %s%s\n", l, nm, m.nrow, m.ncol,
                               static_cast<long long>(m.nnz), static_cast<double>(m.nnz) / m.nrow, m.max_row, m.rpc ? "stream" : "vec", m.rpc, m.lanes,
                               m.valf ? "f32" : "f64", m.cid ? " c16" : "");
    };
    for (size_t l = 0; l < nl; ++l) {
      show("A", l, ctx->amg[l].A); show("P", l, ctx->amg[l].P); show("R", l, ctx->amg[l].R);
      show("Rt", l, ctx->amg[l].Rt); show("GP", l, ctx->amg[l].GP);
    }
  }
  HF_TRY(wire_levels(ctx));
  lap("+ operators on the device");
  ctx->coarse_n = 0;
  if (nl > 1 && coarse_n > 0 && coarse_n <= 4096) {
    const int nc = coarse_n;
    const int ld = (nc + 3) & ~3;
    HF_TRY(dev_alloc(ctx, &ctx->d_coarse_inv, static_cast<size_t>(nc) * ld));
    HF_TRY(dense_inverse(ctx, nc, Ac.ptr.data(), Ac.idx.data(), Ac.val.data(), ctx->d_coarse_inv));
    if (f32) {
      HF_TRY(dev_alloc(ctx, &ctx->d_coarse_inv_f, static_cast<size_t>(nc) * ld));
      hipLaunchKernelGGL(k_to_float, dim3(1024), dim3(256), 0, ctx->stream, static_cast<size_t>(nc) * ld, ctx->d_coarse_inv, ctx->d_coarse_inv_f);
      HF_HIP(hipGetLastError());
    }
    HF_HIP(hipStreamSynchronize(ctx->stream));
    ctx->coarse_ld = ld;
    ctx->coarse_n = nc;
  }
  lap("+ dense inverse");
  ctx->amg_opc = op_complexity;
  ctx->amg_fine_stale = false;
  ctx->amg_ready = true;
  ctx->amg_setup_s = std::chrono::duration<double>(std::chrono::steady_clock::now() - t0).count();
  return HF_OK;
}

int build_amg(hf_ctx* ctx) {
  const auto t0 = std::chrono::steady_clock::now();
  free_amg(ctx);
  amg::Csr A0;
  A0.nrow = A0.ncol = ctx->n;
  A0.ptr.assign(ctx->h_rowptr.begin(), ctx->h_rowptr.end());
  A0.idx.assign(ctx->h_colidx.begin(), ctx->h_colidx.end());
  A0.val.resize(ctx->nnz);
  HF_HIP(copy_sync(ctx, A0.val.data(), ctx->d_A, sizeof(double) * ctx->nnz, hipMemcpyDeviceToHost));
  amg::Hierarchy H;
  amg::Params prm;
  amg_params(ctx, prm);
  auto lap = [&](const char* what) {
    if (prm.verbose) std::fprintf(stderr, "[amg setup] %-28s %.3f s\n", what, std::chrono::duration<double>(std::chrono::steady_clock::now() - t0).count());
  };
  lap("operator downloaded");
  if (!amg::build(std::move(A0), prm, H)) return fail(ctx, HF_ERR_STATE, "AMG set-up failed (non-positive diagonal or singular coarse operator)");
  lap("+ host hierarchy");
  ctx->amg.resize(H.levels.size());
  HF_TRY(upload_host_levels(ctx, H, 0));
  return finish_amg(ctx, H.levels.back().A, H.coarse_n, H.op_complexity, t0);
}

inline bool short_chunks(const DevCsr& m) { return m.nchunks > 0 && m.nnz <= static_cast<int64_t>(m.nchunks) * (7 * TS / 2); }

template <int SM, typename VT>
void launch_stream_t(hf_ctx* c, const DevCsr& m, const VT* val, const double* x, double* y, double* part0, const double* bvec,
                     double* conv_part) {
  const int npart = c->P;
  static const int grid_cap = std::getenv("HEATFLOW_STREAM_GRID") ? std::atoi(std::getenv("HEATFLOW_STREAM_GRID")) : MAXP;
  int grid = std::min(m.nchunks, (SM == 0 && part0 == nullptr) ? std::max(grid_cap, 1) : npart);
  if (grid >= 64) grid &= ~7;
#define HF_STREAM_ARGS2 m.nrow, m.nchunks, m.rpc, m.ptr, m.idx, val, x, y, c->d_scal, part0, bvec, static_cast<const double*>(nullptr), \
                        static_cast<double*>(nullptr), static_cast<double*>(nullptr), conv_part, 0.0, npart, 0
  if (m.cid != nullptr && sizeof(VT) == 4 && short_chunks(m))
    hipLaunchKernelGGL((k_spmv<SM, true, VT, 4>), dim3(grid), dim3(TS), static_cast<size_t>(m.chunk_nnz + m.max_dict) * 8, c->stream,
                       HF_STREAM_ARGS2, ColComp{m.dptr, m.dict, m.cid, m.chunk_nnz, 0});
  else if (m.cid != nullptr)
    hipLaunchKernelGGL((k_spmv<SM, true, VT>), dim3(grid), dim3(TS), static_cast<size_t>(m.chunk_nnz + m.max_dict) * 8, c->stream,
                       HF_STREAM_ARGS2, ColComp{m.dptr, m.dict, m.cid, m.chunk_nnz, 0});
  else
    hipLaunchKernelGGL((k_spmv<SM, false, VT>), dim3(grid), dim3(TS), static_cast<size_t>(m.chunk_nnz) * 8, c->stream,
                       HF_STREAM_ARGS2, ColComp{nullptr, nullptr, nullptr, 0, 0});
#undef HF_STREAM_ARGS2
}

template <int SM>
void launch_stream(hf_ctx* c, const DevCsr& m, const double* x, double* y, double* part0, const double* bvec, double* conv_part) {
  if (m.valf != nullptr) launch_stream_t<SM, float>(c, m, m.valf, x, y, part0, bvec, conv_part);
  else launch_stream_t<SM, double>(c, m, m.val, x, y, part0, bvec, conv_part);
}

template <int VMODE, typename VT>
void launch_vec_t(hf_ctx* c, const DevCsr& m, const VT* val, const double* x, double* y) {
  if (m.rpc > 0) {
    constexpr int SM = VMODE == 0 ? 0 : 6;
    static const int grid_cap = std::getenv("HEATFLOW_STREAM_GRID") ? std::atoi(std::getenv("HEATFLOW_STREAM_GRID")) : MAXP;
    int grid = std::min(m.nchunks, std::max(grid_cap, 1));
    if (grid >= 64) grid &= ~7;
#define HF_STREAM_ARGS m.nrow, m.nchunks, m.rpc, m.ptr, m.idx, val, x, y, c->d_scal, static_cast<double*>(nullptr),                       \
                       static_cast<const double*>(nullptr), static_cast<const double*>(nullptr), static_cast<double*>(nullptr),   \
                       static_cast<double*>(nullptr), static_cast<double*>(nullptr), 0.0, 0, 0
    if (m.cid != nullptr && sizeof(VT) == 4 && short_chunks(m))
      hipLaunchKernelGGL((k_spmv<SM, true, VT, 4>), dim3(grid), dim3(TS), static_cast<size_t>(m.chunk_nnz + m.max_dict) * 8, c->stream,
                         HF_STREAM_ARGS, ColComp{m.dptr, m.dict, m.cid, m.chunk_nnz, 0});
    else if (m.cid != nullptr)
      hipLaunchKernelGGL((k_spmv<SM, true, VT>), dim3(grid), dim3(TS), static_cast<size_t>(m.chunk_nnz + m.max_dict) * 8, c->stream,
                         HF_STREAM_ARGS, ColComp{m.dptr, m.dict, m.cid, m.chunk_nnz, 0});
    else
      hipLaunchKernelGGL((k_spmv<SM, false, VT>), dim3(grid), dim3(TS), static_cast<size_t>(m.chunk_nnz) * 8, c->stream,
                         HF_STREAM_ARGS, ColComp{nullptr, nullptr, nullptr, 0, 0});
#undef HF_STREAM_ARGS
    return;
  }
  if (m.lanes > 64) {
    hipLaunchKernelGGL((k_spmv_row<VMODE, VT>), dim3(std::max(1, std::min(m.nrow, 4096))), dim3(TPB), 0, c->stream, m.nrow, m.ptr,
                       m.idx, val, x, y, c->d_scal);
    return;
  }
  const int lanes = m.lanes;
  const long long threads = static_cast<long long>(m.nrow) * lanes;
  const int grid = static_cast<int>(std::max(1LL, std::min<long long>((threads + TPB - 1) / TPB, 2048)));
#define HF_VEC(L) hipLaunchKernelGGL((k_spmv_vec<L, VMODE, VT>), dim3(grid), dim3(TPB), 0, c->stream, m.nrow, m.ptr, m.idx, val, x, y, c->d_scal)
  switch (lanes) {
    case 4: HF_VEC(4); break;
    case 8: HF_VEC(8); break;
    case 16: HF_VEC(16); break;
    case 32: HF_VEC(32); break;
    default: HF_VEC(64); break;
  }
#undef HF_VEC
}

template <int VMODE>
void launch_vec(hf_ctx* c, const DevCsr& m, const double* x, double* y) {
  if (m.valf != nullptr) launch_vec_t<VMODE, float>(c, m, m.valf, x, y);
  else launch_vec_t<VMODE, double>(c, m, m.val, x, y);
}

enum CyclePart { CYCLE_ALL = 0, CYCLE_FIRST = 1, CYCLE_REST = 2 };
void vcycle(hf_ctx* c, int out_slot, bool test_convergence = false, CyclePart part = CYCLE_ALL) {
  const int nl = static_cast<int>(c->amg.size());
  DevLevel& L0 = c->amg[0];
  if (nl == 1) {
    if (part != CYCLE_REST)
      launch_spmv<4>(c, c->d_A, c->d_z, c->d_z2, c->d_part_rz + out_slot * MAXP, c->d_r, nullptr, nullptr, nullptr, L0.omega);
    return;
  }
  const bool fused0 = L0.GP.nrow > 0;
  if (L0.Rt.nrow > 0 && (fused0 || !c->amg_fine_stale)) {
    if (part != CYCLE_REST) launch_stream<0>(c, L0.Rt, c->d_r, c->amg[1].b, nullptr, nullptr, test_convergence ? c->d_part_zz : nullptr);
  } else {
    if (part != CYCLE_REST)
      launch_spmv<3>(c, c->d_A, c->d_z, c->d_tmp, nullptr, c->d_r, nullptr, nullptr,
                     test_convergence ? c->d_part_zz : nullptr);
    if (part != CYCLE_FIRST) launch_vec<0>(c, L0.R, c->d_tmp, c->amg[1].b);
  }
  if (part == CYCLE_FIRST) return;
  for (int l = 1; l + 1 < nl; ++l) launch_vec<0>(c, c->amg[l].Rt, c->amg[l].b, c->amg[l + 1].b);
  {
    DevLevel& Lc = c->amg[nl - 1];
    if (c->coarse_n > 0) {
      const int g = std::max(1, std::min((Lc.n + 1) / 2, 2048));
      if (c->d_coarse_inv_f != nullptr)
        hipLaunchKernelGGL(k_dense_mv_f32, dim3(g), dim3(TPB), 0, c->stream, Lc.n, c->coarse_ld, c->d_coarse_inv_f, Lc.b, Lc.res, c->d_scal);
      else
        hipLaunchKernelGGL(k_dense_mv, dim3(g), dim3(TPB), 0, c->stream, Lc.n, c->coarse_ld, c->d_coarse_inv, Lc.b, Lc.res, c->d_scal);
    } else {
      const int g = std::max(1, std::min((Lc.n + TPB - 1) / TPB, 1024));
      hipLaunchKernelGGL(k_scale, dim3(g), dim3(TPB), 0, c->stream, Lc.n, Lc.omega, Lc.dinv, Lc.b, Lc.res, c->d_scal);
    }
  }
  for (int l = nl - 2; l >= 1; --l) launch_vec<0>(c, c->amg[l].GP, c->amg[l].cat, c->amg[l].res);
  if (fused0) {
    launch_stream<7>(c, L0.GP, c->d_r, c->d_z2, c->d_part_rz + out_slot * MAXP, c->d_r, nullptr);
    return;
  }
  launch_vec<1>(c, L0.P, c->amg[1].res, c->d_z);
  launch_spmv<4>(c, c->d_A, c->d_z, c->d_z2, c->d_part_rz + out_slot * MAXP, c->d_r, nullptr, nullptr, nullptr, L0.omega);
}

void launch_amg_iteration(hf_ctx* c, double* x, int parity, CyclePart part = CYCLE_ALL) {
  if (part == CYCLE_REST) { vcycle(c, parity ^ 1, true, CYCLE_REST); return; }
  const bool timed = c->prof && c->prof_used < PROF_PAIRS;
  hipEvent_t e0 = timed ? c->prof_ev[2 * c->prof_used] : nullptr, e1 = timed ? c->prof_ev[2 * c->prof_used + 1] : nullptr;
  launch_spmv<9>(c, c->d_A, c->d_z2, c->d_Ap, c->d_part_pAp, nullptr, c->d_p, c->d_part_rz, c->d_part_zz, 0.0, nullptr, e0,
                 e1, parity);
  if (timed) c->prof_used++;
  hipLaunchKernelGGL(k_pcg_update_amg, dim3(c->P), dim3(TPB), 0, c->stream, c->n, c->nchunks, c->P, parity, c->d_scal,
                     c->d_part_pAp, c->d_part_rz, c->d_part_zz, x, c->d_r, c->d_p, c->d_Ap, c->d_dinv,
                     c->amg[0].omega, c->amg[0].GP.nrow > 0 ? static_cast<double*>(nullptr) : c->d_z);
  vcycle(c, parity ^ 1, true, part);
}

inline bool poll_enabled() {
  static const bool on = !(std::getenv("HEATFLOW_POLL") && std::getenv("HEATFLOW_POLL")[0] == '0');
  return on;
}

int reset_scal(hf_ctx* ctx) {
  *ctx->h_scal = Scal{};
  ctx->h_scal->mirror = ctx->d_mirror;
  HF_HIP(hipMemcpyAsync(ctx->d_scal, ctx->h_scal, sizeof(Scal), hipMemcpyHostToDevice, ctx->stream));
  HF_HIP(hipStreamSynchronize(ctx->stream));
  return HF_OK;
}

void harvest_profile(hf_ctx* ctx);

int read_scal(hf_ctx* ctx) {
  HF_HIP(hipMemcpyAsync(ctx->h_scal, ctx->d_scal, sizeof(Scal), hipMemcpyDeviceToHost, ctx->stream));
  HF_HIP(hipStreamSynchronize(ctx->stream));
  harvest_profile(ctx);
  return HF_OK;
}

int wait_tested(hf_ctx* ctx, int k) {
  static const double limit_s = std::getenv("HEATFLOW_POLL_TIMEOUT_S") ? std::atof(std::getenv("HEATFLOW_POLL_TIMEOUT_S")) : 60.0;
  ScalMirror* m = ctx->h_mirror;
  const unsigned ep = ctx->epoch;
  const auto t0 = std::chrono::steady_clock::now();
  auto last_query = t0;
  for (unsigned spin = 1;; ++spin) {
    const int tested = mirror_tested(m, ep);
    const int done = mirror_done(m, ep);
    if (tested >= k || done != 0) break;
    cpu_relax();
    if ((spin & 0x3ff) == 0) {
      const auto now = std::chrono::steady_clock::now();
      if (now - last_query < std::chrono::milliseconds(2)) continue;
      last_query = now;
      if (hipStreamQuery(ctx->stream) == hipSuccess) {
        if (mirror_tested(m, ep) >= k || mirror_done(m, ep) != 0) break;
        return fail(ctx, HF_ERR_HIP, "PCG progress: stream drained before the test of iteration %d ran (%s)", k, hipGetErrorString(hipGetLastError()));
      }
      if (std::chrono::duration<double>(std::chrono::steady_clock::now() - t0).count() > limit_s)
        return fail(ctx, HF_ERR_HIP, "PCG progress: no convergence test within %.0f s (waiting for iteration %d, at %d)", limit_s, k, tested);
    }
  }
  __atomic_thread_fence(__ATOMIC_ACQUIRE);
  ctx->h_scal->iters = m->iters;
  ctx->h_scal->zz = m->zz;
  ctx->h_scal->bn2 = m->bn2;
  ctx->h_scal->done = mirror_done(m, ep);
  return HF_OK;
}

void harvest_profile(hf_ctx* ctx) {
  if (ctx->prof) {
    for (int k = 0; k < ctx->prof_used; ++k) {
      float ms = 0.f;
      const bool ran = !ctx->h_scal->done || (ctx->prof_base + k) < ctx->h_scal->iters;
      if (ran && hipEventElapsedTime(&ms, ctx->prof_ev[2 * k], ctx->prof_ev[2 * k + 1]) == hipSuccess) {
        ctx->prof_spmv_ms += ms;
        ctx->prof_spmv_n += 1;
      }
    }
    ctx->prof_used = 0;
  }
}

int pcg_solve(hf_ctx* ctx, const LinSys& sys, bool use_amg, double rtol, double atol, int max_it, int* pred) {
  static const bool trace_res = std::getenv("HEATFLOW_TRACE_RES") != nullptr;
  ctx->epoch += 1;
  if (!use_amg) {
    launch_spmv<2>(ctx, sys.A, sys.x, ctx->d_r, ctx->d_part_rz, sys.b, ctx->d_z, ctx->d_part_zz, ctx->d_part_bn, 0.0,
                   sys.dinv);
    hipLaunchKernelGGL(k_pcg_begin, dim3(1), dim3(TPB), 0, ctx->stream, ctx->P, rtol, atol, ctx->d_part_zz,
                       ctx->d_part_bn, ctx->d_scal, ctx->epoch);
  } else {
    launch_spmv<5>(ctx, sys.A, sys.x, ctx->d_r, nullptr, sys.b, ctx->d_z, ctx->d_part_zz, ctx->d_part_bn,
                   ctx->amg[0].omega);
    hipLaunchKernelGGL(k_pcg_begin, dim3(1), dim3(TPB), 0, ctx->stream, ctx->P, rtol, atol, ctx->d_part_zz,
                       ctx->d_part_bn, ctx->d_scal, ctx->epoch);
    vcycle(ctx, 0);
  }
  HF_HIP(hipGetLastError());

  int launched = 0;
  if (use_amg && !trace_res && ctx->amg.size() > 1 && poll_enabled()) {
    ctx->prof_base = 0;
    auto finish = [&](int rc) {
      if (ctx->prof) { (void)hipStreamSynchronize(ctx->stream); harvest_profile(ctx); }
      return rc;
    };
    if (*pred <= 0) {
      HF_TRY(wait_tested(ctx, 0));
      if (ctx->h_scal->done == 1) return finish(HF_OK);
    }
    static const bool hold_back = !(std::getenv("HEATFLOW_HOLD_BACK") && std::getenv("HEATFLOW_HOLD_BACK")[0] == '0');
    int burst = std::max(1, std::min(max_it, *pred - 2));
    bool rest_pending = false;
    while (true) {
      if (rest_pending) launch_amg_iteration(ctx, sys.x, (launched - 1) & 1, CYCLE_REST);
      const bool split = hold_back && burst == 1 && launched > 0;
      for (int k = 0; k < burst; ++k) launch_amg_iteration(ctx, sys.x, (launched + k) & 1, split ? CYCLE_FIRST : CYCLE_ALL);
      rest_pending = split;
      launched += burst;
      HF_HIP(hipGetLastError());
      const int rc = wait_tested(ctx, launched);
      if (rc != HF_OK) return finish(rc);
      if (ctx->h_scal->done || launched >= max_it) break;
      burst = 1;
    }
    *pred = ctx->h_scal->iters;
    if (ctx->h_scal->done == 2) return finish(fail(ctx, HF_ERR_NOCONV, "PCG breakdown (p.Ap <= 0) after %d iterations", ctx->h_scal->iters));
    if (!ctx->h_scal->done)
      return finish(fail(ctx, HF_ERR_NOCONV, "PCG not converged in %d iterations (rel. residual %.3e)", ctx->h_scal->iters,
                         std::sqrt(ctx->h_scal->zz / std::max(ctx->h_scal->bn2, 1e-300))));
    return finish(HF_OK);
  }
  if (*pred <= 0) {
    HF_TRY(read_scal(ctx));
    if (ctx->h_scal->done == 1) return HF_OK;
  }
  int burst = std::max(1, std::min(max_it, *pred > 0 ? *pred : (use_amg ? 8 : 32)));
  if (trace_res) burst = 2;
  while (true) {
    ctx->prof_base = launched;
    for (int k = 0; k < burst; ++k) {
      if (use_amg) launch_amg_iteration(ctx, sys.x, (launched + k) & 1);
      else launch_pcg_iteration(ctx, sys, (launched + k) & 1);
    }
    launched += burst;
    HF_HIP(hipGetLastError());
    HF_TRY(read_scal(ctx));
    if (trace_res) std::fprintf(stderr, "[res] it %d rel %.3e\n", ctx->h_scal->iters, std::sqrt(ctx->h_scal->zz / std::max(ctx->h_scal->bn2, 1e-300)));
    if (ctx->h_scal->done) break;
    if (launched >= max_it) break;
    burst = std::max(1, std::min(std::max(use_amg ? 1 : 8, launched / 8), max_it - launched));
    if (trace_res) burst = 2;
  }
  *pred = ctx->h_scal->iters;
  if (ctx->h_scal->done == 2) return fail(ctx, HF_ERR_NOCONV, "PCG breakdown (p.Ap <= 0) after %d iterations", ctx->h_scal->iters);
  if (!ctx->h_scal->done)
    return fail(ctx, HF_ERR_NOCONV, "PCG not converged in %d iterations (rel. residual %.3e)", ctx->h_scal->iters,
                std::sqrt(ctx->h_scal->zz / std::max(ctx->h_scal->bn2, 1e-300)));
  return HF_OK;
}

void proj_clear(hf_ctx* ctx, bool ring_only = false) {
  for (int k = 0; k < (ring_only ? PROJ_MH : PROJ_MT); ++k) ctx->proj.used[k] = false;
  ctx->proj.next = 0;
  ctx->proj.pending = -1;
}

void proj_free(hf_ctx* ctx) {
  proj_clear(ctx);
  for (auto& v : ctx->proj.V) dev_free(&v);
  for (auto& v : ctx->proj.F) dev_free(&v);
  dev_free(&ctx->proj.G); dev_free(&ctx->proj.alpha); dev_free(&ctx->proj.part);
  ctx->proj.ready = false;
}

void free_responses(hf_ctx* ctx) {
  for (auto& r : ctx->resp) dev_free(&r.w);
  ctx->resp.clear();
  ctx->g_hist = 0;
  proj_clear(ctx);
}

int proj_ensure(hf_ctx* ctx) {
  hf_ctx::Proj& Q = ctx->proj;
  if (Q.ready) return HF_OK;
  for (int k = 0; k < PROJ_MT; ++k) {
    HF_TRY(dev_alloc(ctx, &Q.V[k], ctx->n));
    HF_TRY(dev_alloc(ctx, &Q.F[k], ctx->n));
  }
  HF_TRY(dev_alloc(ctx, &Q.G, PROJ_MT * PROJ_MT));
  HF_TRY(dev_alloc(ctx, &Q.alpha, PROJ_MT + 1));
  HF_TRY(dev_alloc(ctx, &Q.part, static_cast<size_t>(2) * PROJ_MT * MAXP));
  HF_HIP(hipMemsetAsync(Q.G, 0, sizeof(double) * PROJ_MT * PROJ_MT, ctx->stream));
  Q.ready = true;
  proj_clear(ctx);
  return HF_OK;
}

ProjVecs proj_active(const hf_ctx* ctx) {
  ProjVecs a{};
  a.m = 0;
  for (int k = 0; k < PROJ_MT; ++k)
    if (ctx->proj.used[k]) { a.V[a.m] = ctx->proj.V[k]; a.slot[a.m] = k; ++a.m; }
  return a;
}

int proj_store(hf_ctx* ctx, int slot, const double* u, const double* rhs) {
  hf_ctx::Proj& Q = ctx->proj;
  hipLaunchKernelGGL(k_copy2, dim3(ctx->P), dim3(TPB), 0, ctx->stream, ctx->n, u, Q.V[slot], rhs, Q.F[slot]);
  if (ctx->nbc > 0)
    hipLaunchKernelGGL(k_zero_entries, dim3((ctx->nbc + 255) / 256), dim3(256), 0, ctx->stream, ctx->nbc, ctx->d_bc_dofs, Q.V[slot]);
  Q.used[slot] = true;
  return HF_OK;
}

void proj_column(hf_ctx* ctx, int slot, const double* f, bool solve) {
  hf_ctx::Proj& Q = ctx->proj;
  const ProjVecs a = proj_active(ctx);
  hipLaunchKernelGGL(k_proj_dots, dim3(ctx->P), dim3(TPB), 0, ctx->stream, ctx->n, a, f, slot >= 0 ? Q.F[slot] : static_cast<const double*>(nullptr),
                     Q.part);
  hipLaunchKernelGGL(k_proj_solve, dim3(1), dim3(PROJ_SOLVE_T), 0, ctx->stream, ctx->P, a, slot, solve ? 1 : 0, Q.part, Q.G, Q.alpha);
}

int solve_response(hf_ctx* ctx, const std::vector<double>& dir, int max_it, double** w_out) {
  double* w = nullptr;
  HF_TRY(dev_alloc(ctx, &w, ctx->n));
  const int nb = ctx->nbc;
  HF_HIP(hipMemsetAsync(w, 0, sizeof(double) * ctx->n, ctx->stream));
  HF_HIP(hipMemsetAsync(ctx->d_b, 0, sizeof(double) * ctx->n, ctx->stream));
  HF_HIP(hipMemcpyAsync(ctx->d_g, dir.data(), sizeof(double) * nb, hipMemcpyHostToDevice, ctx->stream));
  if (ctx->nlift_rows > 0)
    hipLaunchKernelGGL(k_lift, dim3((ctx->nlift_rows + 255) / 256), dim3(256), 0, ctx->stream, ctx->nlift_rows,
                       ctx->d_lift_rows, ctx->d_lift_ptr, ctx->d_lift_bc, ctx->d_lift_val, ctx->d_g, ctx->d_b);
  hipLaunchKernelGGL(k_set_bc, dim3((nb + 255) / 256), dim3(256), 0, ctx->stream, nb, ctx->d_bc_dofs, ctx->d_g, ctx->d_b, w);
  const LinSys sys{ctx->d_A, ctx->d_dinv, w, ctx->d_b};
  const bool use_amg = ctx->precond == 1 && ctx->amg_ready;
  int pred = ctx->pred_iters;
  int rc = pcg_solve(ctx, sys, use_amg, 1e-8, 0.0, max_it, &pred);
  if (rc == HF_ERR_NOCONV && use_amg && ctx->h_scal->done == 2) rc = pcg_solve(ctx, sys, false, 1e-8, 0.0, max_it, &pred);
  if (rc != HF_OK) { dev_free(&w); return rc; }
  ctx->resp_solves += 1;
  *w_out = w;
  if (ctx->start_kind == 3 && ctx->proj.ready) {
    const int slot = PROJ_MH + static_cast<int>(ctx->resp.size());
    HF_TRY(proj_store(ctx, slot, w, ctx->d_b));
    proj_column(ctx, slot, nullptr, false);
  }
  return HF_OK;
}

int prepare_response(hf_ctx* ctx, const double* g_new, int max_it, RespArgs* ra) {
  const int nb = ctx->nbc;
  ra->k = 0;
  std::vector<double> rem(nb);
  double nrm2 = 0.0, gn2 = 0.0;
  for (int q = 0; q < nb; ++q) {
    rem[q] = (g_new[q] - ctx->h_g0[q]) - (ctx->h_g0[q] - ctx->h_g1[q]);
    nrm2 += rem[q] * rem[q];
    gn2 += g_new[q] * g_new[q];
  }
  if (!(nrm2 > 0.0)) return HF_OK;
  for (size_t k = 0; k < ctx->resp.size(); ++k) {
    const std::vector<double>& d = ctx->resp[k].dir;
    double c = 0.0;
    for (int q = 0; q < nb; ++q) c += d[q] * rem[q];
    for (int q = 0; q < nb; ++q) rem[q] -= c * d[q];
    ra->c[k] = c;
    ra->w[k] = ctx->resp[k].w;
  }
  double rn2 = 0.0;
  for (int q = 0; q < nb; ++q) rn2 += rem[q] * rem[q];
  if (rn2 > 1e-12 * nrm2 && nrm2 > 1e-18 * gn2 && ctx->resp.size() < static_cast<size_t>(MAXRESP)) {
    const double rn = std::sqrt(rn2);
    hf_ctx::BcResponse nr;
    nr.dir.resize(nb);
    for (int q = 0; q < nb; ++q) nr.dir[q] = rem[q] / rn;
    const int rc = solve_response(ctx, nr.dir, max_it, &nr.w);
    if (rc == HF_ERR_HIP) return rc;
    if (rc == HF_OK) {
      ra->c[ctx->resp.size()] = rn;
      ra->w[ctx->resp.size()] = nr.w;
      ctx->resp.push_back(std::move(nr));
    } else {
      ctx->start_kind = 1;
    }
  }
  ra->k = static_cast<int>(ctx->resp.size());
  return HF_OK;
}

void launch_rhs(hf_ctx* ctx) {
  if (ctx->have_load)
    launch_spmv<10>(ctx, ctx->d_M, ctx->d_u, ctx->d_b, nullptr, nullptr, nullptr, nullptr, nullptr, ctx->dt, ctx->d_load);
  else
    launch_spmv<0>(ctx, ctx->d_M, ctx->d_u, ctx->d_b);
}

void launch_rhs_bdf2(hf_ctx* ctx, bool extrap) {
  const double* um1 = ctx->bdf_hist ? ctx->d_uprev : ctx->d_u;
  if (ctx->have_load) {
    if (extrap) launch_spmv<15>(ctx, ctx->d_M, ctx->d_u, ctx->d_b, nullptr, um1, ctx->d_ustart, nullptr, nullptr, ctx->dt, ctx->d_load);
    else launch_spmv<14>(ctx, ctx->d_M, ctx->d_u, ctx->d_b, nullptr, um1, ctx->d_ustart, nullptr, nullptr, ctx->dt, ctx->d_load);
  } else {
    if (extrap) launch_spmv<13>(ctx, ctx->d_M, ctx->d_u, ctx->d_b, nullptr, um1, ctx->d_ustart);
    else launch_spmv<12>(ctx, ctx->d_M, ctx->d_u, ctx->d_b, nullptr, um1, ctx->d_ustart);
  }
}

int kt_revalue(hf_ctx* ctx, const double* u, const double* uprev) {
  const int cap = (ctx->max_blk_nnz + 1) & ~1;
  const int capd = ctx->rg_max_dict;
  const size_t sm = static_cast<size_t>(cap) * 8 + static_cast<size_t>(capd) * 16 + static_cast<size_t>(capd + (capd & 1)) * 8 +
                    (RBA + 4) * 4 + (static_cast<size_t>(cap) / 8 + 3) * 16;
  if (ctx->kt.grid == 0) {
    const void* fn = reinterpret_cast<const void*>(&k_assemble_rows_kT);
    if (sm > 64 * 1024) HF_HIP(hipFuncSetAttribute(fn, hipFuncAttributeMaxDynamicSharedMemorySize, static_cast<int>(sm)));
    int per_cu = 0, ncu = 0;
    HF_HIP(hipOccupancyMaxActiveBlocksPerMultiprocessor(&per_cu, fn, RBA, sm));
    HF_HIP(hipDeviceGetAttribute(&ncu, hipDeviceAttributeMultiprocessorCount, ctx->dev));
    ctx->kt.grid = std::max(1, std::min(ctx->nblk_a, std::max(1, per_cu) * std::max(1, ncu)));
  }
  hipLaunchKernelGGL(k_assemble_rows_kT, dim3(ctx->kt.grid), dim3(RBA), sm, ctx->stream, ctx->nblk_a, cap, capd, ctx->d_rowptr,
                     ctx->d_rg_hdr, reinterpret_cast<const uint4*>(ctx->d_rg_ell), reinterpret_cast<const uint4*>(ctx->d_rg_cid),
                     ctx->d_rg_zrb, ctx->d_rg_dict, ctx->kt.hdr, ctx->kt.vals, ctx->d_kappa_rg, ctx->d_rhoc_rg, ctx->dt, u, uprev,
                     ctx->d_A);
  if (ctx->nbc > 0) {
    if (ctx->nlift > 0)
      hipLaunchKernelGGL(k_take_lift, dim3((ctx->nlift + 255) / 256), dim3(256), 0, ctx->stream, ctx->nlift, ctx->d_lift_slot, ctx->d_A,
                         ctx->d_lift_val);
    hipLaunchKernelGGL(k_bc_rows, dim3((ctx->nbc + 255) / 256), dim3(256), 0, ctx->stream, ctx->nbc, ctx->d_bc_dofs, ctx->d_rowptr,
                       ctx->d_colidx, ctx->d_A);
  }
  hipLaunchKernelGGL(k_dinv, dim3((ctx->n + 255) / 256), dim3(256), 0, ctx->stream, ctx->n, ctx->d_rowptr, ctx->d_colidx, ctx->d_A,
                     ctx->d_dinv);
  HF_HIP(hipGetLastError());
  return HF_OK;
}

int step_solve(hf_ctx* ctx, double rtol, double atol, int max_it) {
  const LinSys sys{ctx->d_A, ctx->d_dinv, ctx->d_u, ctx->d_b};
  const bool use_amg = ctx->precond == 1 && ctx->amg_ready;
  int rc = pcg_solve(ctx, sys, use_amg, rtol, atol, max_it, &ctx->pred_iters);
  if (rc == HF_ERR_NOCONV && use_amg && ctx->h_scal->done == 2) {
    ctx->amg_fallbacks += 1;
    int pred = 0;
    rc = pcg_solve(ctx, sys, false, rtol, atol, max_it, &pred);
  }
  return rc;
}

int step_device(hf_ctx* ctx, const double* g_host, const double* g_dev, double rtol, double atol, int max_it, bool last = true) {
  const int nb = ctx->nbc;
  RespArgs ra{};
  ra.k = 0;
  const bool kt = ctx->kt.on;
  const int kind = kt && ctx->start_kind >= 2 ? 1 : ctx->start_kind;
  const bool projected = kind == 3;
  const bool bdf2 = ctx->scheme == HF_TIME_BDF2;
  if (projected) HF_TRY(proj_ensure(ctx));
  const bool hist_ok = nb > 0 && ctx->extrapolate && ctx->have_prev && ctx->g_hist >= 2;
  if (kind >= 2 && hist_ok && !(bdf2 && kind == 2)) HF_TRY(prepare_response(ctx, g_host, max_it, &ra));
  const int sweeps = kt ? ctx->kt.picard : 1;
  const bool track = kt && last;
  if (kt) {
    const double* um1 = bdf2 && ctx->bdf_hist ? ctx->d_uprev : nullptr;
    HF_TRY(kt_revalue(ctx, ctx->d_u, um1));
    if (ctx->precond == 1 && ctx->amg_ready) ctx->amg_fine_stale = true;
    if (track && sweeps == 1)
      hipLaunchKernelGGL(k_eval_state, dim3(ctx->P), dim3(TPB), 0, ctx->stream, ctx->n, ctx->d_u, um1, ctx->kt.pic);
  }
  const double* g = g_dev ? g_dev : ctx->d_g;
  if (nb > 0 && !g_dev) HF_HIP(hipMemcpyAsync(ctx->d_g, g_host, sizeof(double) * nb, hipMemcpyHostToDevice, ctx->stream));
  if (bdf2 && (projected || !ctx->extrapolate)) {
    launch_rhs_bdf2(ctx, false);
    std::swap(ctx->d_uprev, ctx->d_ustart);
    ctx->bdf_hist = true;
    ctx->have_prev = true;
  } else if (bdf2) {
    launch_rhs_bdf2(ctx, true);
    HF_HIP(hipMemcpyAsync(ctx->d_uprev, ctx->d_u, sizeof(double) * ctx->n, hipMemcpyDeviceToDevice, ctx->stream));
    HF_HIP(hipMemcpyAsync(ctx->d_u, ctx->d_ustart, sizeof(double) * ctx->n, hipMemcpyDeviceToDevice, ctx->stream));
    ctx->bdf_hist = true;
    ctx->have_prev = true;
  } else if (projected) {
    launch_rhs(ctx);
    ctx->have_prev = true;
  } else if (ctx->extrapolate && ctx->have_prev) {
    if (ctx->have_load)
      launch_spmv<11>(ctx, ctx->d_M, ctx->d_u, ctx->d_b, nullptr, ctx->d_uprev, ctx->d_ustart, nullptr, nullptr, ctx->dt, ctx->d_load);
    else
      launch_spmv<8>(ctx, ctx->d_M, ctx->d_u, ctx->d_b, nullptr, ctx->d_uprev, ctx->d_ustart);
    HF_HIP(hipMemcpyAsync(ctx->d_uprev, ctx->d_u, sizeof(double) * ctx->n, hipMemcpyDeviceToDevice, ctx->stream));
    if (ra.k > 0)
      hipLaunchKernelGGL(k_start_vector, dim3(ctx->P), dim3(TPB), 0, ctx->stream, ctx->n, ctx->d_ustart, ra, ctx->d_u);
    else
      HF_HIP(hipMemcpyAsync(ctx->d_u, ctx->d_ustart, sizeof(double) * ctx->n, hipMemcpyDeviceToDevice, ctx->stream));
  } else {
    launch_rhs(ctx);
    if (ctx->extrapolate) {
      HF_HIP(hipMemcpyAsync(ctx->d_uprev, ctx->d_u, sizeof(double) * ctx->n, hipMemcpyDeviceToDevice, ctx->stream));
      ctx->have_prev = true;
    }
  }
  const bool combine = projected && proj_active(ctx).m > 0;
  if (sweeps > 1)
    HF_HIP(hipMemcpyAsync(ctx->kt.b0, ctx->d_b, sizeof(double) * ctx->n, hipMemcpyDeviceToDevice, ctx->stream));
  if (nb > 0) {
    if (ctx->nlift_rows > 0)
      hipLaunchKernelGGL(k_lift, dim3((ctx->nlift_rows + 255) / 256), dim3(256), 0, ctx->stream, ctx->nlift_rows,
                         ctx->d_lift_rows, ctx->d_lift_ptr, ctx->d_lift_bc, ctx->d_lift_val, g, ctx->d_b);
    if (!combine)
      hipLaunchKernelGGL(k_set_bc, dim3((nb + 255) / 256), dim3(256), 0, ctx->stream, nb, ctx->d_bc_dofs, g,
                         ctx->d_b, ctx->d_u);
  }
  if (combine) {
    hf_ctx::Proj& Q = ctx->proj;
    proj_column(ctx, Q.pending, ctx->d_b, true);
    Q.pending = -1;
    hipLaunchKernelGGL(k_proj_combine, dim3(ctx->P), dim3(TPB), 0, ctx->stream, ctx->n, proj_active(ctx), Q.alpha, ctx->d_u);
    if (nb > 0)
      hipLaunchKernelGGL(k_set_bc, dim3((nb + 255) / 256), dim3(256), 0, ctx->stream, nb, ctx->d_bc_dofs, g, ctx->d_b, ctx->d_u);
  }
  int rc = step_solve(ctx, rtol, atol, max_it);
  if (kt) {
    int total = ctx->h_scal->iters;
    for (int k = 2; k <= sweeps && rc == HF_OK; ++k) {
      if (track && k == sweeps)
        HF_HIP(hipMemcpyAsync(ctx->kt.pic, ctx->d_u, sizeof(double) * ctx->n, hipMemcpyDeviceToDevice, ctx->stream));
      HF_TRY(kt_revalue(ctx, ctx->d_u, nullptr));
      HF_HIP(hipMemcpyAsync(ctx->d_b, ctx->kt.b0, sizeof(double) * ctx->n, hipMemcpyDeviceToDevice, ctx->stream));
      if (nb > 0) {
        if (ctx->nlift_rows > 0)
          hipLaunchKernelGGL(k_lift, dim3((ctx->nlift_rows + 255) / 256), dim3(256), 0, ctx->stream, ctx->nlift_rows,
                             ctx->d_lift_rows, ctx->d_lift_ptr, ctx->d_lift_bc, ctx->d_lift_val, g, ctx->d_b);
        hipLaunchKernelGGL(k_set_bc, dim3((nb + 255) / 256), dim3(256), 0, ctx->stream, nb, ctx->d_bc_dofs, g, ctx->d_b, ctx->d_u);
      }
      rc = step_solve(ctx, rtol, atol, max_it);
      total += ctx->h_scal->iters;
    }
    ctx->h_scal->iters = total;
    if (rc == HF_OK && track) {
      HF_HIP(hipMemsetAsync(ctx->kt.change, 0, sizeof(unsigned long long), ctx->stream));
      hipLaunchKernelGGL(k_max_abs_diff, dim3(ctx->P), dim3(TPB), 0, ctx->stream, ctx->n, ctx->d_u, ctx->kt.pic, ctx->kt.change);
      ctx->kt.have_change = true;
    }
  }
  if (rc == HF_OK && projected) {
    hf_ctx::Proj& Q = ctx->proj;
    HF_TRY(proj_store(ctx, Q.next, ctx->d_u, ctx->d_b));
    Q.pending = Q.next;
    Q.next = (Q.next + 1) % PROJ_MH;
  }
  if (rc == HF_OK && nb > 0) {
    ctx->h_g1.swap(ctx->h_g0);
    ctx->h_g0.assign(g_host, g_host + nb);
    if (ctx->g_hist < 2) ctx->g_hist += 1;
  }
  return rc;
}

int ensure_samples(hf_ctx* ctx, int ns) {
  if (ns <= ctx->samp_cap) return HF_OK;
  HF_TRY(dev_alloc(ctx, &ctx->d_samp_idx, ns));
  HF_TRY(dev_alloc(ctx, &ctx->d_samp, ns));
  ctx->samp_cap = ns;
  return HF_OK;
}

int build_lift(hf_ctx* ctx) {
  const int32_t n = ctx->n, nbc = ctx->nbc;
  std::vector<int32_t> dofs(nbc);
  HF_HIP(copy_sync(ctx, dofs.data(), ctx->d_bc_dofs, sizeof(int32_t) * nbc, hipMemcpyDeviceToHost));
  std::vector<int32_t> bc_index(n, -1);
  for (int32_t q = 0; q < nbc; ++q) bc_index[dofs[q]] = q;
  std::vector<int32_t> rows;
  for (int32_t q = 0; q < nbc; ++q) {
    const int32_t j = dofs[q];
    for (int32_t k = ctx->h_rowptr[j]; k < ctx->h_rowptr[j + 1]; ++k) {
      const int32_t i = ctx->h_colidx[k];
      if (bc_index[i] < 0) rows.push_back(i);
    }
  }
  std::sort(rows.begin(), rows.end());
  rows.erase(std::unique(rows.begin(), rows.end()), rows.end());
  std::vector<int32_t> ptr(rows.size() + 1, 0), lbc, lslot;
  for (size_t r = 0; r < rows.size(); ++r) {
    const int32_t i = rows[r];
    for (int32_t k = ctx->h_rowptr[i]; k < ctx->h_rowptr[i + 1]; ++k) {
      const int32_t q = bc_index[ctx->h_colidx[k]];
      if (q >= 0) { lbc.push_back(q); lslot.push_back(k); }
    }
    ptr[r + 1] = static_cast<int32_t>(lbc.size());
  }
  ctx->nlift_rows = static_cast<int32_t>(rows.size());
  ctx->nlift = static_cast<int32_t>(lbc.size());
  HF_TRY(dev_alloc(ctx, &ctx->d_lift_rows, rows.size()));
  HF_TRY(dev_alloc(ctx, &ctx->d_lift_ptr, ptr.size()));
  HF_TRY(dev_alloc(ctx, &ctx->d_lift_bc, lbc.size()));
  HF_TRY(dev_alloc(ctx, &ctx->d_lift_slot, lslot.size()));
  HF_TRY(dev_alloc(ctx, &ctx->d_lift_val, lbc.size()));
  if (!rows.empty()) HF_HIP(copy_sync(ctx, ctx->d_lift_rows, rows.data(), sizeof(int32_t) * rows.size(), hipMemcpyHostToDevice));
  HF_HIP(copy_sync(ctx, ctx->d_lift_ptr, ptr.data(), sizeof(int32_t) * ptr.size(), hipMemcpyHostToDevice));
  if (!lbc.empty()) {
    HF_HIP(copy_sync(ctx, ctx->d_lift_bc, lbc.data(), sizeof(int32_t) * lbc.size(), hipMemcpyHostToDevice));
    HF_HIP(copy_sync(ctx, ctx->d_lift_slot, lslot.data(), sizeof(int32_t) * lslot.size(), hipMemcpyHostToDevice));
  }
  return HF_OK;
}

}
```

Measured before the change: 730.4 million.

## Fuse projected-start step: RHS, projection dots, initial guess and residual into SpMV

Adds two SpMV modes for the projected-start path. Mode 16 builds the right-hand side, including the Dirichlet and lift corrections from a row-tag array, while accumulating the projection dot products. Mode 17 forms the projected initial guess on the fly and computes the first PCG residual and preconditioned vector, so pcg_solve can skip its starting SpMV. Storing the pending projection vector is deferred (lazy), and k_spmv takes a larger StepFuse argument and more register and shared-memory state, which may lower occupancy for every mode.

New measurement: 718.2 million (median of 3 runs). -1.7%, worse.

```diff
diff --git a/heatflow_amd/csrc/heatflow_hip.hip b/heatflow_amd/csrc/heatflow_hip.hip
--- a/heatflow_amd/csrc/heatflow_hip.hip
+++ b/heatflow_amd/csrc/heatflow_hip.hip
@@ -569,7 +569,7 @@
   dev_free(&ctx->d_zr); dev_free(&ctx->d_elem); dev_free(&ctx->d_kappa); dev_free(&ctx->d_rhoc);
   dev_free(&ctx->d_rowptr); dev_free(&ctx->d_colidx); dev_free(&ctx->d_cdict_ptr); dev_free(&ctx->d_cdict); dev_free(&ctx->d_cid); dev_free(&ctx->d_blk_eptr); dev_free(&ctx->d_blk_cptr); dev_free(&ctx->d_blk_ent); dev_free(&ctx->d_rg_hdr); dev_free(&ctx->d_rg_ell); dev_free(&ctx->d_rg_cid); dev_free(&ctx->d_rg_dict); dev_free(&ctx->d_rg_zrb); dev_free(&ctx->d_kappa_rg); dev_free(&ctx->d_rhoc_rg); dev_free(&ctx->d_M); dev_free(&ctx->d_A); dev_free(&ctx->d_dinv);
   dev_free(&ctx->d_bc_dofs); dev_free(&ctx->d_g); dev_free(&ctx->d_lift_rows); dev_free(&ctx->d_lift_ptr);
-  dev_free(&ctx->d_lift_bc); dev_free(&ctx->d_lift_slot); dev_free(&ctx->d_lift_val);
+  dev_free(&ctx->d_lift_bc); dev_free(&ctx->d_lift_slot); dev_free(&ctx->d_lift_val); dev_free(&ctx->d_rowtag);
   dev_free(&ctx->d_uprev); dev_free(&ctx->d_ustart);
   dev_free(&ctx->d_u); dev_free(&ctx->d_b); dev_free(&ctx->d_r); dev_free(&ctx->d_p); dev_free(&ctx->d_Ap);
   free_batch(ctx); free_batch_state(ctx->fluxb); free_batch_cols(ctx); free_amg(ctx); free_responses(ctx); proj_free(ctx); dev_free(&ctx->d_z); dev_free(&ctx->d_z2);
@@ -718,6 +718,7 @@
   HF_TRY(dev_alloc(ctx, &ctx->d_g, n_bc));
   if (n_bc > 0) HF_HIP(copy_sync(ctx, ctx->d_bc_dofs, dofs, sizeof(int32_t) * n_bc, hipMemcpyHostToDevice));
   HF_TRY(build_lift(ctx));
+  ctx->rowtag_ok = false;
   free_amg(ctx);
   free_responses(ctx);
   ctx->assembled = false;
diff --git a/heatflow_amd/csrc/hf_context.hpp b/heatflow_amd/csrc/hf_context.hpp
--- a/heatflow_amd/csrc/hf_context.hpp
+++ b/heatflow_amd/csrc/hf_context.hpp
@@ -137,6 +137,8 @@
   int32_t nlift_rows = 0, nlift = 0;
   int32_t *d_lift_rows = nullptr, *d_lift_ptr = nullptr, *d_lift_bc = nullptr, *d_lift_slot = nullptr;
   double* d_lift_val = nullptr;
+  int32_t* d_rowtag = nullptr;
+  bool rowtag_ok = false;
   double *d_u = nullptr, *d_b = nullptr, *d_r = nullptr, *d_p = nullptr, *d_Ap = nullptr;
   double *d_uprev = nullptr, *d_ustart = nullptr;
   bool have_prev = false;
@@ -152,6 +154,7 @@
     double *V[PROJ_MT] = {nullptr}, *F[PROJ_MT] = {nullptr};
     bool used[PROJ_MT] = {false};
     int next = 0, pending = -1;
+    bool lazy = false;
     double *G = nullptr, *alpha = nullptr, *part = nullptr;
     bool ready = false;
   } proj;
diff --git a/heatflow_amd/csrc/hf_kernels.hpp b/heatflow_amd/csrc/hf_kernels.hpp
--- a/heatflow_amd/csrc/hf_kernels.hpp
+++ b/heatflow_amd/csrc/hf_kernels.hpp
@@ -661,6 +661,13 @@
   u[dofs[q]] = g[q];
 }
 
+__global__ void k_rowtag(int nbc, const int32_t* __restrict__ dofs, int nrows, const int32_t* __restrict__ rows,
+                         int32_t* __restrict__ tag) {
+  const int q = blockIdx.x * blockDim.x + threadIdx.x;
+  if (q < nbc) tag[dofs[q]] = -(q + 1);
+  else if (q < nbc + nrows) tag[rows[q - nbc]] = q - nbc + 1;
+}
+
 __global__ void k_gather(int ns, const int32_t* __restrict__ idx, const double* __restrict__ u,
                          double* __restrict__ out) {
   const int q = blockIdx.x * blockDim.x + threadIdx.x;
@@ -697,6 +704,20 @@
 __device__ __forceinline__ void mirror_breakdown(ScalMirror* m, unsigned epoch) {
   if (m != nullptr) __hip_atomic_store(&m->done_st, mirror_stamp(epoch, 2), __ATOMIC_RELEASE, __HIP_MEMORY_SCOPE_SYSTEM);
 }
+
+struct ProjVecs { const double* V[PROJ_MT]; int slot[PROJ_MT]; int m; };
+struct StepFuse {
+  const int32_t* tag;
+  const double* g;
+  const int32_t* lptr; const int32_t* lbc; const double* lval;
+  ProjVecs a;
+  int pend;
+  double* vpend;
+  const double* fpend;
+  double* part;
+  const double* alpha;
+  double* u;
+};
 
 struct ColComp { const int32_t* dptr; const int32_t* dict; const uint16_t* id; int xd_off; int own; };
 
@@ -742,12 +763,25 @@
                                               const double* __restrict__ dinv, double* __restrict__ pvec,
                                               double* __restrict__ part1, double* __restrict__ part2, double w,
                                               int npart ,
-                                              int parity, ColComp comp) {
+                                              int parity, ColComp comp, StepFuse sf) {
   extern __shared__ double sprod[];
   __shared__ double s4[TS / 64];
   __shared__ int s_own;
+  __shared__ double s_dot[TS / 64][2 * PROJ_MT];
   constexpr bool BDF = MODE >= 12 && MODE <= 15;
-  auto opnd = [&](int c) { return BDF ? bdf2_operand(x[c], bvec[c]) : x[c]; };
+  constexpr bool OWNX = MODE == 4 || MODE == 8 || MODE == 9 || MODE == 11 || MODE == 16 || MODE == 17;
+  double al[PROJ_MT];
+#pragma unroll
+  for (int k = 0; k < PROJ_MT; ++k) al[k] = (MODE == 17 && k < sf.a.m) ? sf.alpha[sf.a.slot[k]] : 0.0;
+  auto x0_at = [&](int c) {
+    double s = 0.0;
+#pragma unroll
+    for (int k = 0; k < PROJ_MT; ++k)
+      if (k < sf.a.m) s += al[k] * sf.a.V[k][c];
+    const int t = sf.tag[c];
+    return t < 0 ? sf.g[-t - 1] : s;
+  };
+  auto opnd = [&](int c) { return MODE == 17 ? x0_at(c) : BDF ? bdf2_operand(x[c], bvec[c]) : x[c]; };
   if ((MODE == 3 || MODE == 4 || MODE == 6 || MODE == 9) && scal->done) return;
   if ((MODE == 0 || MODE == 7) && scal != nullptr && scal->done) return;
   double acc0 = 0.0, acc1 = 0.0, acc2 = 0.0;
@@ -795,17 +829,22 @@
   const int tpr = (MODE == 0 || MODE == 6 || MODE == 7) ? TS / rpc : 1;
   const int prel = static_cast<int>(threadIdx.x) / tpr;
   const int psub = static_cast<int>(threadIdx.x) % tpr;
-  struct RowOps { double b, d, y, p, x; };
+  struct RowOps { double b, d, y, p, x; int t; };
   auto row_operands = [&](int prc, bool from_slice) {
-    RowOps e{0.0, 0.0, 0.0, 0.0, 0.0};
-    if (MODE == 2 || MODE == 3 || MODE == 4 || MODE == 5 || MODE == 7 || MODE == 8 || MODE == 11 || MODE == 13 || MODE == 15) e.b = bvec[prc];
-    if (MODE == 2 || MODE == 4 || MODE == 5 || MODE == 10 || MODE == 11 || MODE == 14 || MODE == 15) e.d = dinv[prc];
+    RowOps e{0.0, 0.0, 0.0, 0.0, 0.0, 0};
+    if (MODE == 2 || MODE == 3 || MODE == 4 || MODE == 5 || MODE == 17 || MODE == 7 || MODE == 8 || MODE == 11 || MODE == 13 || MODE == 15) e.b = bvec[prc];
+    if (MODE == 2 || MODE == 4 || MODE == 5 || MODE == 17 || MODE == 10 || MODE == 11 || MODE == 14 || MODE == 15) e.d = dinv[prc];
     if (MODE == 6 || (MODE == 9 && !first9)) e.y = y[prc];
     if (MODE == 9 && !first9) e.p = pvec[prc];
-    if ((MODE == 4 || MODE == 8 || MODE == 9 || MODE == 11) && !from_slice) e.x = x[prc];
+    if ((MODE == 4 || MODE == 8 || MODE == 9 || MODE == 11 || MODE == 16) && !from_slice) e.x = x[prc];
+    if (MODE == 17 && !from_slice) e.x = x0_at(prc);
     if (BDF) e.x = x[prc];
+    if (MODE == 16) e.t = sf.tag[prc];
     return e;
   };
+  double f16_b = 0.0, f16_v = 0.0;
+  if (MODE == 16)
+    for (int q = threadIdx.x; q < (TS / 64) * 2 * PROJ_MT; q += TS) (&s_dot[0][0])[q] = 0.0;
   auto rows_phase = [&](bool pin, int prow, int pa, int pb, const RowOps& e) {
     if ((MODE == 0 || MODE == 6 || MODE == 7) && tpr > 1) {
       double s = 0.0;
@@ -858,6 +897,27 @@
       } else if (BDF) {
         y[row] = (MODE == 14 || MODE == 15) ? s + w * e.d : s;
         pvec[row] = (MODE == 13 || MODE == 15) ? 2.0 * e.x - e.b : e.x;
+      } else if (MODE == 16) {
+        double bi = s;
+        if (e.t > 0) {
+          double q = 0.0;
+          for (int k = sf.lptr[e.t - 1]; k < sf.lptr[e.t]; ++k) q += sf.lval[k] * sf.g[sf.lbc[k]];
+          bi -= q;
+        } else if (e.t < 0) {
+          bi = sf.g[-e.t - 1];
+        }
+        y[row] = bi;
+        const double vi = e.t < 0 ? 0.0 : e.x;
+        if (sf.pend >= 0) sf.vpend[row] = vi;
+        f16_b = bi;
+        f16_v = vi;
+      } else if (MODE == 17) {
+        const double ri = e.b - s;
+        y[row] = ri;
+        pvec[row] = w * e.d * ri;
+        sf.u[row] = e.x;
+        acc1 += (e.d * ri) * (e.d * ri);
+        acc2 += (e.d * e.b) * (e.d * e.b);
       } else {
         const double api = first9 ? s : s + beta * e.y;
         const double pi = first9 ? e.x : e.x + beta * e.p;
@@ -866,6 +926,24 @@
         acc0 += pi * api;
       }
     }
+  };
+  auto dots16 = [&](bool pin, int prc) {
+    if (MODE != 16) return;
+    const double fp = sf.fpend != nullptr ? sf.fpend[prc] : 0.0;
+    double vk[PROJ_MT];
+#pragma unroll
+    for (int k = 0; k < PROJ_MT; ++k) vk[k] = (k < sf.a.m && sf.a.slot[k] != sf.pend) ? sf.a.V[k][prc] : 0.0;
+    const double bi = pin ? f16_b : 0.0, fpi = pin ? fp : 0.0;
+    const int lane = threadIdx.x & 63, wave = threadIdx.x >> 6;
+#pragma unroll
+    for (int k = 0; k < PROJ_MT; ++k)
+      if (k < sf.a.m) {
+        const double v = pin ? (sf.a.slot[k] == sf.pend ? f16_v : vk[k]) : 0.0;
+        double th = v * bi, tg = v * fpi;
+#pragma unroll
+        for (int o = 32; o > 0; o >>= 1) { th += __shfl_down(th, o, 64); tg += __shfl_down(tg, o, 64); }
+        if (lane == 0) { s_dot[wave][2 * k] += th; s_dot[wave][2 * k + 1] += tg; }
+      }
   };
   if (PIPELINED) {
     struct Bounds { int k0, k1, d0, d1; };
@@ -915,7 +993,7 @@
         const int i = static_cast<int>(threadIdx.x) + u * TS;
         if (i < nd) {
           xd[i] = x0[u];
-          if ((MODE == 4 || MODE == 8 || MODE == 9 || MODE == 11) && c0[u] == r0) s_own = i;
+          if (OWNX && c0[u] == r0) s_own = i;
         }
       }
       for (int i = threadIdx.x + HF_STAGE_U * TS; i < nd; i += HF_STAGE_U * TS) {
@@ -929,12 +1007,12 @@
         for (int u = 0; u < HF_STAGE_U; ++u)
           if (i + u * TS < nd) {
             xd[i + u * TS] = xv[u];
-            if ((MODE == 4 || MODE == 8 || MODE == 9 || MODE == 11) && c[u] == r0) s_own = i + u * TS;
+            if (OWNX && c[u] == r0) s_own = i + u * TS;
           }
       }
       __syncthreads();
       HF_STAMP(stamp_at); ++stamp_at;
-      if ((MODE == 4 || MODE == 8 || MODE == 9 || MODE == 11) && comp.own && pin) e.x = xd[s_own + (prow - r0)];
+      if (OWNX && comp.own && pin) e.x = xd[s_own + (prow - r0)];
 #pragma unroll
       for (int u = 0; u < UN; ++u) {
         const int kk = k0 + static_cast<int>(threadIdx.x) + u * TS;
@@ -957,6 +1035,7 @@
       __syncthreads();
       HF_STAMP(stamp_at); ++stamp_at;
       rows_phase(pin, prow, pa, pb, e);
+      dots16(pin, prc);
       __syncthreads();
       HF_STAMP(stamp_at); ++stamp_at;
       cur = nxt;
@@ -999,12 +1078,12 @@
         for (int u = 0; u < HF_STAGE_U; ++u)
           if (i + u * TS < nd) {
             xd[i + u * TS] = xv[u];
-            if ((MODE == 4 || MODE == 8 || MODE == 9 || MODE == 11) && c[u] == r0) s_own = i + u * TS;
+            if (OWNX && c[u] == r0) s_own = i + u * TS;
           }
       }
       __syncthreads();
       HF_STAMP(stamp_at); ++stamp_at;
-      if ((MODE == 4 || MODE == 8 || MODE == 9 || MODE == 11) && comp.own && pin) e.x = xd[s_own + (prow - r0)];
+      if (OWNX && comp.own && pin) e.x = xd[s_own + (prow - r0)];
       while (k < k1) {
         const int kn = k + HF_UNROLL * TS;
         double vn[HF_UNROLL];
@@ -1042,6 +1121,7 @@
     __syncthreads();
     HF_STAMP(stamp_at); ++stamp_at;
     rows_phase(pin, prow, pa, pb, e);
+    dots16(pin, min(prow, r1 - 1));
     __syncthreads();
     HF_STAMP(stamp_at); ++stamp_at;
   }
@@ -1053,7 +1133,17 @@
       for (int q = blockIdx.x + gridDim.x; q < npart; q += gridDim.x) part0[q] = 0.0;
     }
   }
-  if (MODE == 2 || MODE == 5) {
+  if (MODE == 16) {
+    __syncthreads();
+    const int q = threadIdx.x;
+    if (q < 2 * sf.a.m) {
+      double t = s_dot[0][q];
+      for (int wv = 1; wv < TS / 64; ++wv) t += s_dot[wv][q];
+      sf.part[q * MAXP + blockIdx.x] = t;
+      for (int b = blockIdx.x + gridDim.x; b < npart; b += gridDim.x) sf.part[q * MAXP + b] = 0.0;
+    }
+  }
+  if (MODE == 2 || MODE == 5 || MODE == 17) {
     const double t1 = block_sum<TS / 64>(acc1, s4);
     const double t2 = block_sum<TS / 64>(acc2, s4);
     if (threadIdx.x == 0) {
@@ -1196,7 +1286,6 @@
   }
 }
 
-struct ProjVecs { const double* V[PROJ_MT]; int slot[PROJ_MT]; int m; };
 
 __global__ __launch_bounds__(TPB) void k_proj_dots(int n, ProjVecs a, const double* __restrict__ f, const double* __restrict__ Fnew,
                                                    double* __restrict__ part ) {
diff --git a/heatflow_amd/csrc/hf_pattern.hpp b/heatflow_amd/csrc/hf_pattern.hpp
--- a/heatflow_amd/csrc/hf_pattern.hpp
+++ b/heatflow_amd/csrc/hf_pattern.hpp
@@ -373,11 +373,11 @@
 void launch_spmv(hf_ctx* c, const VT* vals, const double* x, double* y, double* part0 = nullptr,
                  const double* bvec = nullptr, double* pvec = nullptr, double* part1 = nullptr,
                  double* part2 = nullptr, double w = 0.0, const double* dinv = nullptr, hipEvent_t ev_start = nullptr,
-                 hipEvent_t ev_stop = nullptr, int parity = 0) {
+                 hipEvent_t ev_stop = nullptr, int parity = 0, const StepFuse& sf = StepFuse{}) {
   const ColComp comp{c->d_cdict_ptr, c->d_cdict, c->d_cid, c->max_chunk_nnz_s, c->cdict_own ? 1 : 0};
 #define HF_SPMV_ARGS c->n, c->nchunks_s, static_cast<int>(SRPC), static_cast<const int32_t*>(c->d_rowptr),                    \
                      static_cast<const int32_t*>(c->d_colidx), vals, x, y, (MODE == 0 ? nullptr : c->d_scal), part0, bvec,  \
-                     dinv ? dinv : static_cast<const double*>(c->d_dinv), pvec, part1, part2, w, c->P, parity, comp
+                     dinv ? dinv : static_cast<const double*>(c->d_dinv), pvec, part1, part2, w, c->P, parity, comp, sf
   const std::uint32_t smem = static_cast<std::uint32_t>(spmv_smem_bytes(c));
   if (c->c16) {
     if (ev_start != nullptr) hipExtLaunchKernelGGL((k_spmv<MODE, true, VT, HF_SPMV_UN>), dim3(c->Ps), dim3(TS), smem, c->stream, ev_start, ev_stop, 0u, HF_SPMV_ARGS);
diff --git a/heatflow_amd/csrc/hf_solver.hpp b/heatflow_amd/csrc/hf_solver.hpp
--- a/heatflow_amd/csrc/hf_solver.hpp
+++ b/heatflow_amd/csrc/hf_solver.hpp
@@ -264,13 +264,13 @@
                         static_cast<double*>(nullptr), static_cast<double*>(nullptr), conv_part, 0.0, npart, 0
   if (m.cid != nullptr && sizeof(VT) == 4 && short_chunks(m))
     hipLaunchKernelGGL((k_spmv<SM, true, VT, 4>), dim3(grid), dim3(TS), static_cast<size_t>(m.chunk_nnz + m.max_dict) * 8, c->stream,
-                       HF_STREAM_ARGS2, ColComp{m.dptr, m.dict, m.cid, m.chunk_nnz, 0});
+                       HF_STREAM_ARGS2, ColComp{m.dptr, m.dict, m.cid, m.chunk_nnz, 0}, StepFuse{});
   else if (m.cid != nullptr)
     hipLaunchKernelGGL((k_spmv<SM, true, VT>), dim3(grid), dim3(TS), static_cast<size_t>(m.chunk_nnz + m.max_dict) * 8, c->stream,
-                       HF_STREAM_ARGS2, ColComp{m.dptr, m.dict, m.cid, m.chunk_nnz, 0});
+                       HF_STREAM_ARGS2, ColComp{m.dptr, m.dict, m.cid, m.chunk_nnz, 0}, StepFuse{});
   else
     hipLaunchKernelGGL((k_spmv<SM, false, VT>), dim3(grid), dim3(TS), static_cast<size_t>(m.chunk_nnz) * 8, c->stream,
-                       HF_STREAM_ARGS2, ColComp{nullptr, nullptr, nullptr, 0, 0});
+                       HF_STREAM_ARGS2, ColComp{nullptr, nullptr, nullptr, 0, 0}, StepFuse{});
 #undef HF_STREAM_ARGS2
 }
 
@@ -292,13 +292,13 @@
                        static_cast<double*>(nullptr), static_cast<double*>(nullptr), 0.0, 0, 0
     if (m.cid != nullptr && sizeof(VT) == 4 && short_chunks(m))
       hipLaunchKernelGGL((k_spmv<SM, true, VT, 4>), dim3(grid), dim3(TS), static_cast<size_t>(m.chunk_nnz + m.max_dict) * 8, c->stream,
-                         HF_STREAM_ARGS, ColComp{m.dptr, m.dict, m.cid, m.chunk_nnz, 0});
+                         HF_STREAM_ARGS, ColComp{m.dptr, m.dict, m.cid, m.chunk_nnz, 0}, StepFuse{});
     else if (m.cid != nullptr)
       hipLaunchKernelGGL((k_spmv<SM, true, VT>), dim3(grid), dim3(TS), static_cast<size_t>(m.chunk_nnz + m.max_dict) * 8, c->stream,
-                         HF_STREAM_ARGS, ColComp{m.dptr, m.dict, m.cid, m.chunk_nnz, 0});
+                         HF_STREAM_ARGS, ColComp{m.dptr, m.dict, m.cid, m.chunk_nnz, 0}, StepFuse{});
     else
       hipLaunchKernelGGL((k_spmv<SM, false, VT>), dim3(grid), dim3(TS), static_cast<size_t>(m.chunk_nnz) * 8, c->stream,
-                         HF_STREAM_ARGS, ColComp{nullptr, nullptr, nullptr, 0, 0});
+                         HF_STREAM_ARGS, ColComp{nullptr, nullptr, nullptr, 0, 0}, StepFuse{});
 #undef HF_STREAM_ARGS
     return;
   }
@@ -449,7 +449,7 @@
   }
 }
 
-int pcg_solve(hf_ctx* ctx, const LinSys& sys, bool use_amg, double rtol, double atol, int max_it, int* pred) {
+int pcg_solve(hf_ctx* ctx, const LinSys& sys, bool use_amg, double rtol, double atol, int max_it, int* pred, bool started = false) {
   static const bool trace_res = std::getenv("HEATFLOW_TRACE_RES") != nullptr;
   ctx->epoch += 1;
   if (!use_amg) {
@@ -458,8 +458,9 @@
     hipLaunchKernelGGL(k_pcg_begin, dim3(1), dim3(TPB), 0, ctx->stream, ctx->P, rtol, atol, ctx->d_part_zz,
                        ctx->d_part_bn, ctx->d_scal, ctx->epoch);
   } else {
-    launch_spmv<5>(ctx, sys.A, sys.x, ctx->d_r, nullptr, sys.b, ctx->d_z, ctx->d_part_zz, ctx->d_part_bn,
-                   ctx->amg[0].omega);
+    if (!started)
+      launch_spmv<5>(ctx, sys.A, sys.x, ctx->d_r, nullptr, sys.b, ctx->d_z, ctx->d_part_zz, ctx->d_part_bn,
+                     ctx->amg[0].omega);
     hipLaunchKernelGGL(k_pcg_begin, dim3(1), dim3(TPB), 0, ctx->stream, ctx->P, rtol, atol, ctx->d_part_zz,
                        ctx->d_part_bn, ctx->d_scal, ctx->epoch);
     vcycle(ctx, 0);
@@ -532,6 +533,7 @@
   for (int k = 0; k < (ring_only ? PROJ_MH : PROJ_MT); ++k) ctx->proj.used[k] = false;
   ctx->proj.next = 0;
   ctx->proj.pending = -1;
+  ctx->proj.lazy = false;
 }
 
 void proj_free(hf_ctx* ctx) {
@@ -571,6 +573,16 @@
   for (int k = 0; k < PROJ_MT; ++k)
     if (ctx->proj.used[k]) { a.V[a.m] = ctx->proj.V[k]; a.slot[a.m] = k; ++a.m; }
   return a;
+}
+
+void proj_settle(hf_ctx* ctx) {
+  hf_ctx::Proj& Q = ctx->proj;
+  if (Q.lazy && Q.pending >= 0) {
+    (void)hipMemcpyAsync(Q.V[Q.pending], ctx->d_u, sizeof(double) * ctx->n, hipMemcpyDeviceToDevice, ctx->stream);
+    if (ctx->nbc > 0)
+      hipLaunchKernelGGL(k_zero_entries, dim3((ctx->nbc + 255) / 256), dim3(256), 0, ctx->stream, ctx->nbc, ctx->d_bc_dofs, Q.V[Q.pending]);
+  }
+  Q.lazy = false;
 }
 
 int proj_store(hf_ctx* ctx, int slot, const double* u, const double* rhs) {
@@ -610,6 +622,7 @@
   ctx->resp_solves += 1;
   *w_out = w;
   if (ctx->start_kind == 3 && ctx->proj.ready) {
+    proj_settle(ctx);
     const int slot = PROJ_MH + static_cast<int>(ctx->resp.size());
     HF_TRY(proj_store(ctx, slot, w, ctx->d_b));
     proj_column(ctx, slot, nullptr, false);
@@ -705,14 +718,74 @@
   return HF_OK;
 }
 
-int step_solve(hf_ctx* ctx, double rtol, double atol, int max_it) {
-  const LinSys sys{ctx->d_A, ctx->d_dinv, ctx->d_u, ctx->d_b};
+int step_solve(hf_ctx* ctx, double rtol, double atol, int max_it, const double* b = nullptr, bool started = false) {
+  const LinSys sys{ctx->d_A, ctx->d_dinv, ctx->d_u, b != nullptr ? b : ctx->d_b};
   const bool use_amg = ctx->precond == 1 && ctx->amg_ready;
-  int rc = pcg_solve(ctx, sys, use_amg, rtol, atol, max_it, &ctx->pred_iters);
+  int rc = pcg_solve(ctx, sys, use_amg, rtol, atol, max_it, &ctx->pred_iters, started && use_amg);
   if (rc == HF_ERR_NOCONV && use_amg && ctx->h_scal->done == 2) {
     ctx->amg_fallbacks += 1;
     int pred = 0;
     rc = pcg_solve(ctx, sys, false, rtol, atol, max_it, &pred);
+  }
+  return rc;
+}
+
+inline bool step_fuse_enabled() {
+  static const bool on = !(std::getenv("HEATFLOW_STEP_FUSE") && std::getenv("HEATFLOW_STEP_FUSE")[0] == '0');
+  return on;
+}
+
+int ensure_rowtag(hf_ctx* ctx) {
+  if (ctx->rowtag_ok) return HF_OK;
+  HF_TRY(dev_alloc(ctx, &ctx->d_rowtag, ctx->n));
+  HF_HIP(hipMemsetAsync(ctx->d_rowtag, 0, sizeof(int32_t) * ctx->n, ctx->stream));
+  const int tot = ctx->nbc + ctx->nlift_rows;
+  if (tot > 0)
+    hipLaunchKernelGGL(k_rowtag, dim3((tot + 255) / 256), dim3(256), 0, ctx->stream, ctx->nbc, ctx->d_bc_dofs, ctx->nlift_rows,
+                       ctx->d_lift_rows, ctx->d_rowtag);
+  HF_HIP(hipGetLastError());
+  ctx->rowtag_ok = true;
+  return HF_OK;
+}
+
+int step_fused(hf_ctx* ctx, const double* g, double rtol, double atol, int max_it) {
+  hf_ctx::Proj& Q = ctx->proj;
+  HF_TRY(ensure_rowtag(ctx));
+  const int nb = ctx->nbc;
+  const ProjVecs act = proj_active(ctx);
+  StepFuse sf{};
+  sf.tag = ctx->d_rowtag;
+  sf.g = g;
+  sf.lptr = ctx->d_lift_ptr;
+  sf.lbc = ctx->d_lift_bc;
+  sf.lval = ctx->d_lift_val;
+  sf.a = act;
+  sf.pend = Q.pending;
+  sf.vpend = Q.pending >= 0 ? Q.V[Q.pending] : nullptr;
+  sf.fpend = Q.pending >= 0 ? Q.F[Q.pending] : nullptr;
+  sf.part = Q.part;
+  double* b = Q.F[Q.next];
+  launch_spmv<16>(ctx, ctx->d_M, ctx->d_u, b, nullptr, nullptr, nullptr, nullptr, nullptr, 0.0, nullptr, nullptr, nullptr, 0, sf);
+  Q.lazy = false;
+  bool started = false;
+  if (act.m > 0) {
+    hipLaunchKernelGGL(k_proj_solve, dim3(1), dim3(PROJ_SOLVE_T), 0, ctx->stream, ctx->P, act, Q.pending, 1, Q.part, Q.G, Q.alpha);
+    Q.pending = -1;
+    sf.alpha = Q.alpha;
+    sf.u = ctx->d_u;
+    launch_spmv<17>(ctx, ctx->d_A, ctx->d_u, ctx->d_r, nullptr, b, ctx->d_z, ctx->d_part_zz, ctx->d_part_bn, ctx->amg[0].omega,
+                    nullptr, nullptr, nullptr, 0, sf);
+    started = true;
+  } else {
+    hipLaunchKernelGGL(k_set_bc, dim3((nb + 255) / 256), dim3(256), 0, ctx->stream, nb, ctx->d_bc_dofs, g, b, ctx->d_u);
+  }
+  HF_HIP(hipGetLastError());
+  const int rc = step_solve(ctx, rtol, atol, max_it, b, started);
+  if (rc == HF_OK) {
+    Q.used[Q.next] = true;
+    Q.pending = Q.next;
+    Q.next = (Q.next + 1) % PROJ_MH;
+    Q.lazy = true;
   }
   return rc;
 }
@@ -730,6 +803,9 @@
   if (kind >= 2 && hist_ok && !(bdf2 && kind == 2)) HF_TRY(prepare_response(ctx, g_host, max_it, &ra));
   const int sweeps = kt ? ctx->kt.picard : 1;
   const bool track = kt && last;
+  const bool fuse = projected && !bdf2 && !kt && !ctx->have_load && nb > 0 && ctx->precond == 1 && ctx->amg_ready &&
+                    step_fuse_enabled();
+  if (!fuse) proj_settle(ctx);
   if (kt) {
     const double* um1 = bdf2 && ctx->bdf_hist ? ctx->d_uprev : nullptr;
     HF_TRY(kt_revalue(ctx, ctx->d_u, um1));
@@ -739,6 +815,16 @@
   }
   const double* g = g_dev ? g_dev : ctx->d_g;
   if (nb > 0 && !g_dev) HF_HIP(hipMemcpyAsync(ctx->d_g, g_host, sizeof(double) * nb, hipMemcpyHostToDevice, ctx->stream));
+  if (fuse) {
+    ctx->have_prev = true;
+    const int rc = step_fused(ctx, g, rtol, atol, max_it);
+    if (rc == HF_OK) {
+      ctx->h_g1.swap(ctx->h_g0);
+      ctx->h_g0.assign(g_host, g_host + nb);
+      if (ctx->g_hist < 2) ctx->g_hist += 1;
+    }
+    return rc;
+  }
   if (bdf2 && (projected || !ctx->extrapolate)) {
     launch_rhs_bdf2(ctx, false);
     std::swap(ctx->d_uprev, ctx->d_ustart);
```
